# ria8651/octree-tracer

Hardware: AMD Instinct MI355X
Metric: Mrays/sec at 1920x1080, depth-16 SVO; achieved HBM GB/s vs peak (higher is better)
Workload: dtype f32+u32

## Files before the change

include/svo_hip.h:

```cpp
#ifndef SVO_HIP_H
#define SVO_HIP_H

#include <stddef.h>
#include <stdint.h>

#ifdef __cplusplus
extern "C" {
#endif

#define SVO_VOXEL_OFFSET 134217728u

typedef enum svo_status {
    SVO_OK = 0,
    SVO_ERR_ARG = -1,
    SVO_ERR_HIP = -2,
    SVO_ERR_STATE = -3,
    SVO_ERR_NO_DEVICE = -4,
    SVO_ERR_COMM = -5,
    SVO_ERR_CAP = -6
} svo_status;

#define SVO_F_PAUSE_ADAPTIVE 1u
#define SVO_F_SHOW_STEPS 2u
#define SVO_F_SHOW_HITS 4u
#define SVO_F_SHADOWS 8u
#define SVO_F_MISC_BOOL 16u

typedef struct svo_uniforms {
    float camera[16];
    float camera_inverse[16];
    float dimensions[4];
    float sun_dir[4];
    uint32_t flags;
    float misc_value;
} svo_uniforms;

typedef struct svo_hit {
    uint32_t voxel_index;
    float t;
    uint32_t steps_depth_hit;
    uint32_t packed_normal;
} svo_hit;

typedef struct svo_ctx svo_ctx;

#define SVO_VARIANT_RESTART 0
#define SVO_VARIANT_STACK 1

typedef enum svo_option {
    SVO_OPT_VARIANT = 0,
    SVO_OPT_TIMING = 1,
    SVO_OPT_GRID_BLOCKS = 2,
    SVO_OPT_REFILL_MIN = 3,
    SVO_OPT_STRIP_ITEMS = 4,
    SVO_OPT_DYNAMIC_STRIPS = 5,
    SVO_OPT_SCHEDULE = 8,
    SVO_OPT_TREE_DEPTH = 9,
    SVO_OPT_BLOCK_SHAPE = 10,
    SVO_OPT_DEBUG_BUFFER = 7,
    SVO_OPT_SCAN_CLEARS_COUNTERS = 11,
    SVO_OPT_FUSED_SHADOWS = 12,
    SVO_OPT_PAIR_TABLE = 13,
    SVO_OPT_CULL = 14,
    SVO_OPT_CAMERA_SHORTCUT = 15,
    SVO_OPT_SCHEDULE_MOTION = 16,
    SVO_OPT_PRIO_STEPS = 6
} svo_option;

int svo_device_count(void);
int svo_ctx_create(int hip_device, svo_ctx **out);
int svo_ctx_destroy(svo_ctx *ctx);
int svo_ctx_set_stream(svo_ctx *ctx, void *hip_stream, int use_own);
int svo_set_option(svo_ctx *ctx, int option, int64_t value);
const char *svo_last_error(const svo_ctx *ctx);
int svo_sync(svo_ctx *ctx);

int svo_nodes_alloc(svo_ctx *ctx, size_t capacity_words);
int svo_nodes_bind_device(svo_ctx *ctx, uint32_t *device_words, size_t capacity_words);
int svo_nodes_share(svo_ctx *ctx, svo_ctx *owner);
int svo_nodes_invalidate(svo_ctx *ctx);
int svo_nodes_write(svo_ctx *ctx, size_t word_offset, const uint32_t *host_words, size_t n);
int svo_nodes_scatter(svo_ctx *ctx, const uint32_t *indices, const uint32_t *host_words, size_t n);
int svo_nodes_read(svo_ctx *ctx, size_t word_offset, uint32_t *host_words, size_t n);
int svo_nodes_device_ptr(svo_ctx *ctx, uint32_t **out, size_t *capacity_words);

int svo_buffer_alloc(svo_ctx *ctx, size_t bytes, void **device_out);
int svo_buffer_free(svo_ctx *ctx, void *device_ptr);
int svo_buffer_read(svo_ctx *ctx, const void *device_ptr, void *host_out, size_t bytes);
int svo_buffer_write(svo_ctx *ctx, void *device_dst, const void *host_src, size_t bytes);

int svo_set_uniforms(svo_ctx *ctx, const svo_uniforms *u);

int svo_render(svo_ctx *ctx, uint32_t width, uint32_t height, uint32_t x0, uint32_t y0,
               uint32_t tile_w, uint32_t tile_h, svo_hit *hits_out, uint32_t *rgba_out);
int svo_render_host(svo_ctx *ctx, uint32_t width, uint32_t height, uint32_t x0, uint32_t y0,
                    uint32_t tile_w, uint32_t tile_h, svo_hit *hits_out, uint32_t *rgba_out);
int svo_render_tiles(svo_ctx *ctx, uint32_t width, uint32_t height, uint32_t tile_w,
                     uint32_t tile_h, uint32_t first_tile, uint32_t tile_stride,
                     svo_hit *hits_out, uint32_t *rgba_out);
int svo_render_secondary(svo_ctx *ctx, uint32_t width, uint32_t height, uint32_t x0, uint32_t y0,
                         uint32_t tile_w, uint32_t tile_h, uint32_t n_secondary, svo_hit *primary_out,
                         svo_hit *secondary_out);
int svo_render_tiles_secondary(svo_ctx *ctx, uint32_t width, uint32_t height, uint32_t tile_w,
                               uint32_t tile_h, uint32_t first_tile, uint32_t tile_stride,
                               uint32_t n_secondary, svo_hit *primary_out, svo_hit *secondary_out);
int svo_assemble_tiles(svo_ctx *ctx, const svo_hit *gathered, uint32_t world, uint32_t n_pad, uint32_t width,
                       uint32_t height, uint32_t tile_w, uint32_t tile_h, svo_hit *frame_out);
int svo_pack_records(svo_ctx *ctx, const svo_hit *records, size_t n, uint32_t *wire_out);
int svo_assemble_tiles_packed(svo_ctx *ctx, const uint32_t *gathered_wire, uint32_t world, uint32_t n_pad, uint32_t width,
                              uint32_t height, uint32_t tile_w, uint32_t tile_h, svo_hit *frame_out);
#define SVO_COMM_ID_BYTES 128
int svo_comm_unique_id(uint8_t id_out[SVO_COMM_ID_BYTES]);
int svo_comm_init_rank(svo_ctx *ctx, const uint8_t id[SVO_COMM_ID_BYTES], int world, int rank);
int svo_comm_init_all(int n, svo_ctx *const *ctxs);
int svo_comm_destroy(svo_ctx *ctx);
int svo_gather_frame(svo_ctx *ctx, const void *send, size_t bytes, void *recv_on_root, int root);
int svo_gather_wait(svo_ctx *ctx);
int svo_gather_frame_all(int n, svo_ctx *const *ctxs, const void *const *send, size_t bytes, void *recv_on_root, int root);

int svo_assemble_tiles_rgba(svo_ctx *ctx, const uint32_t *gathered_rgba, uint32_t world, uint32_t n_pad, uint32_t width,
                            uint32_t height, uint32_t tile_w, uint32_t tile_h, uint32_t *rgba_frame_out);

int svo_trace_rays(svo_ctx *ctx, const float *rays, size_t n_rays, svo_hit *hits_out);

int svo_last_render_ms(svo_ctx *ctx, float *ms);
int svo_timing_collect(svo_ctx *ctx, float *ms_out, size_t cap, size_t *n_out);

int svo_diag_gather(svo_ctx *ctx, uint32_t stride_bytes, uint32_t n_loads);

int svo_diag_strip_classes(svo_ctx *ctx, uint8_t *host_out, size_t n_strips);

int svo_scan_dispatch(svo_ctx *ctx, uint32_t node_length);
int svo_scan_read(svo_ctx *ctx, uint32_t *sub, uint32_t *n_sub, uint32_t *unsub, uint32_t *n_unsub,
                  size_t capacity);

struct svo_cpu_octree;
struct svo_world;
typedef struct svo_proc_params {
    float pos[3];
    uint32_t base_depth;
    uint32_t chunk_depth;
    uint64_t max_nodes;
} svo_proc_params;
int svo_proc_generate_chunk(svo_ctx *ctx, const svo_proc_params *params, struct svo_cpu_octree **out);
int svo_world_generate(svo_ctx *ctx, struct svo_world *w, uint32_t world_depth, uint32_t chunk_depth);
int svo_proc_sdf(svo_ctx *ctx, const float *xyz, size_t n, float *out);
int svo_proc_classify(svo_ctx *ctx, const svo_proc_params *params, uint8_t *cells_out);
#define SVO_PROC_TIMES 10
int svo_proc_timing(svo_ctx *ctx, float ms_out[SVO_PROC_TIMES]);

typedef struct svo_build_params {
    uint32_t depth;
    uint32_t default_colour;
    uint64_t max_words;
} svo_build_params;
int svo_nodes_build(svo_ctx *ctx, const uint32_t *xyz, const uint32_t *colours, size_t n, const svo_build_params *p,
                    uint64_t *n_words_out);
int svo_nodes_build_dense(svo_ctx *ctx, const uint32_t *grid, const svo_build_params *p, uint64_t *n_words_out);
#define SVO_BUILD_TIMES 6
int svo_build_timing(svo_ctx *ctx, float ms_out[SVO_BUILD_TIMES]);

typedef struct svo_edit_params {
    uint32_t depth;
    uint32_t default_colour;
    uint64_t n_words;
    uint64_t max_words;
} svo_edit_params;
int svo_nodes_edit(svo_ctx *ctx, const uint32_t *xyz, const uint32_t *colours, size_t n, const svo_edit_params *p,
                   uint64_t *n_words_out);
#define SVO_EDIT_TIMES 6
int svo_edit_timing(svo_ctx *ctx, float ms_out[SVO_EDIT_TIMES]);

#define SVO_COMPACT_PRUNE_EMPTY 1u
typedef struct svo_compact_params {
    uint32_t flags;
    uint32_t reserved;
    uint64_t n_words;
} svo_compact_params;
int svo_nodes_compact(svo_ctx *ctx, const svo_compact_params *p, uint32_t *perm_out_dev , uint64_t *n_words_out);
#define SVO_COMPACT_TIMES 6
int svo_compact_timing(svo_ctx *ctx, float ms_out[SVO_COMPACT_TIMES]);

#define SVO_LIST_EXPAND 1u
typedef struct svo_list_params {
    uint32_t flags;
    uint32_t depth;
    uint64_t n_words;
    uint64_t max_voxels;
} svo_list_params;
int svo_nodes_list_voxels(svo_ctx *ctx, const svo_list_params *p, uint32_t *xyz_out_dev, uint32_t *value_out_dev,
                          uint32_t *level_out_dev , uint64_t *n_out);
#define SVO_LIST_TIMES 5
int svo_list_timing(svo_ctx *ctx, float ms_out[SVO_LIST_TIMES]);

#define SVO_SAMPLE_FINER   (1u << 28)
#define SVO_SAMPLE_OUTSIDE (1u << 29)
#define SVO_SAMPLE_BROKEN  (1u << 30)
typedef struct svo_sample_params {
    uint32_t flags;
    uint32_t depth;
    uint64_t n_words;
} svo_sample_params;
int svo_nodes_sample(svo_ctx *ctx, const svo_sample_params *p, const uint32_t *xyz_dev, size_t n,
                     uint32_t *value_out_dev, uint32_t *level_out_dev , uint32_t *index_out_dev );
int svo_nodes_sample_dense(svo_ctx *ctx, const svo_sample_params *p, const uint32_t origin[3], const uint32_t size[3],
                           uint32_t *grid_out_dev);
#define SVO_SAMPLE_TIMES 2
int svo_sample_timing(svo_ctx *ctx, float ms_out[SVO_SAMPLE_TIMES]);

typedef struct svo_voxelize_params {
    uint32_t depth;
    uint32_t flags;
    uint32_t default_colour;
    uint32_t n_vertices;
// ... 51 lines not shown
```

octree-tracer_amd/_lib.py:

```python
import ctypes as C
import os

import torch

_HERE = os.path.dirname(os.path.abspath(__file__))
LIB_PATH = os.environ.get("SVO_HIP_LIB") or os.path.join(_HERE, "libsvo_hip.so")


class Uniforms(C.Structure):
    _fields_ = [
        ("camera", C.c_float * 16),
        ("camera_inverse", C.c_float * 16),
        ("dimensions", C.c_float * 4),
        ("sun_dir", C.c_float * 4),
        ("flags", C.c_uint32),
        ("misc_value", C.c_float),
    ]


class TerrainParams(C.Structure):
    _fields_ = [
        ("seed", C.c_uint32),
        ("max_depth", C.c_uint32),
        ("cam", C.c_float * 3),
# ... 49 lines not shown
class SampleParams(C.Structure):
    _fields_ = [
        ("flags", C.c_uint32),
        ("depth", C.c_uint32),
        ("n_words", C.c_uint64),
    ]


class VoxelizeParams(C.Structure):
    _fields_ = [
        ("depth", C.c_uint32),
        ("flags", C.c_uint32),
        ("default_colour", C.c_uint32),
        ("n_vertices", C.c_uint32),
        ("max_voxels", C.c_uint64),
    ]


class ChunkBuildParams(C.Structure):
    _fields_ = [
        ("depth", C.c_uint32),
        ("world_depth", C.c_uint32),
        ("default_colour", C.c_uint32),
        ("max_nodes", C.c_uint64),
    ]


class AdaptiveResult(C.Structure):
    _fields_ = [
        ("n_sub", C.c_uint32),
        ("n_unsub", C.c_uint32),
        ("chunks_loaded", C.c_uint64),
        ("length", C.c_uint64),
        ("n_removed", C.c_uint32),
        ("removed", C.POINTER(C.c_uint32)),
    ]


vp, sz, u32, u64, i64, f32 = C.c_void_p, C.c_size_t, C.c_uint32, C.c_uint64, C.c_int64, C.c_float
cp = C.c_char_p
fp = C.POINTER(C.c_float)

DEVICE_SIGNATURES = {
    "svo_device_count": (C.c_int, ()),
    "svo_buffer_alloc": (C.c_int, (vp, sz, C.POINTER(vp))),
    "svo_buffer_free": (C.c_int, (vp, vp)),
    "svo_buffer_read": (C.c_int, (vp, vp, vp, sz)),
    "svo_ctx_create": (C.c_int, (C.c_int, C.POINTER(vp))),
    "svo_ctx_destroy": (C.c_int, (vp,)),
    "svo_ctx_set_stream": (C.c_int, (vp, vp, C.c_int)),
    "svo_set_option": (C.c_int, (vp, C.c_int, i64)),
    "svo_last_error": (cp, (vp,)),
    "svo_sync": (C.c_int, (vp,)),
    "svo_nodes_alloc": (C.c_int, (vp, sz)),
    "svo_nodes_bind_device": (C.c_int, (vp, vp, sz)),
    "svo_nodes_write": (C.c_int, (vp, sz, vp, sz)),
    "svo_nodes_scatter": (C.c_int, (vp, vp, vp, sz)),
    "svo_nodes_read": (C.c_int, (vp, sz, vp, sz)),
    "svo_nodes_device_ptr": (C.c_int, (vp, C.POINTER(vp), C.POINTER(sz))),
    "svo_nodes_share": (C.c_int, (vp, vp)),
    "svo_nodes_invalidate": (C.c_int, (vp,)),
    "svo_comm_unique_id": (C.c_int, (vp,)),
    "svo_comm_init_rank": (C.c_int, (vp, vp, C.c_int, C.c_int)),
    "svo_comm_init_all": (C.c_int, (C.c_int, C.POINTER(vp))),
    "svo_comm_destroy": (C.c_int, (vp,)),
    "svo_gather_frame": (C.c_int, (vp, vp, sz, vp, C.c_int)),
    "svo_gather_wait": (C.c_int, (vp,)),
    "svo_gather_frame_all": (C.c_int, (C.c_int, C.POINTER(vp), C.POINTER(vp), sz, vp, C.c_int)),
    "svo_set_uniforms": (C.c_int, (vp, C.POINTER(Uniforms))),
    "svo_render": (C.c_int, (vp, u32, u32, u32, u32, u32, u32, vp, vp)),
    "svo_render_host": (C.c_int, (vp, u32, u32, u32, u32, u32, u32, vp, vp)),
    "svo_render_tiles": (C.c_int, (vp, u32, u32, u32, u32, u32, u32, vp, vp)),
    "svo_render_secondary": (C.c_int, (vp, u32, u32, u32, u32, u32, u32, u32, vp, vp)),
    "svo_render_tiles_secondary": (C.c_int, (vp, u32, u32, u32, u32, u32, u32, u32, vp, vp)),
    "svo_assemble_tiles": (C.c_int, (vp, vp, u32, u32, u32, u32, u32, u32, vp)),
    "svo_assemble_tiles_packed": (C.c_int, (vp, vp, u32, u32, u32, u32, u32, u32, vp)),
    "svo_assemble_tiles_rgba": (C.c_int, (vp, vp, u32, u32, u32, u32, u32, u32, vp)),
    "svo_pack_records": (C.c_int, (vp, vp, sz, vp)),
    "svo_trace_rays": (C.c_int, (vp, vp, sz, vp)),
    "svo_last_render_ms": (C.c_int, (vp, fp)),
    "svo_timing_collect": (C.c_int, (vp, fp, sz, C.POINTER(sz))),
    "svo_diag_gather": (C.c_int, (vp, u32, u32)),
    "svo_diag_strip_classes": (C.c_int, (vp, vp, sz)),
    "svo_scan_dispatch": (C.c_int, (vp, u32)),
    "svo_scan_read": (C.c_int, (vp, vp, C.POINTER(u32), vp, C.POINTER(u32), sz)),
    "svo_proc_generate_chunk": (C.c_int, (vp, C.POINTER(ProcParams), C.POINTER(vp))),
    "svo_world_generate": (C.c_int, (vp, vp, u32, u32)),
    "svo_proc_sdf": (C.c_int, (vp, vp, sz, vp)),
    "svo_proc_classify": (C.c_int, (vp, C.POINTER(ProcParams), vp)),
    "svo_proc_timing": (C.c_int, (vp, fp)),
    "svo_nodes_build": (C.c_int, (vp, vp, vp, sz, C.POINTER(BuildParams), C.POINTER(u64))),
    "svo_nodes_build_dense": (C.c_int, (vp, vp, C.POINTER(BuildParams), C.POINTER(u64))),
    "svo_buffer_write": (C.c_int, (vp, vp, vp, sz)),
    "svo_build_timing": (C.c_int, (vp, fp)),
    "svo_cpu_octree_build": (C.c_int, (vp, vp, vp, sz, C.POINTER(ChunkBuildParams), C.POINTER(vp))),
    "svo_world_build": (C.c_int, (vp, vp, vp, vp, sz, C.POINTER(ChunkBuildParams))),
    "svo_world_build_timing": (C.c_int, (vp, fp)),
    "svo_nodes_edit": (C.c_int, (vp, vp, vp, sz, C.POINTER(EditParams), C.POINTER(u64))),
    "svo_edit_timing": (C.c_int, (vp, fp)),
    "svo_nodes_compact": (C.c_int, (vp, C.POINTER(CompactParams), vp, C.POINTER(u64))),
    "svo_compact_timing": (C.c_int, (vp, fp)),
    "svo_nodes_list_voxels": (C.c_int, (vp, C.POINTER(ListParams), vp, vp, vp, C.POINTER(u64))),
    "svo_list_timing": (C.c_int, (vp, fp)),
    "svo_nodes_sample": (C.c_int, (vp, C.POINTER(SampleParams), vp, sz, vp, vp, vp)),
    "svo_nodes_sample_dense": (C.c_int, (vp, C.POINTER(SampleParams), C.POINTER(u32), C.POINTER(u32), vp)),
    "svo_sample_timing": (C.c_int, (vp, fp)),
    "svo_mesh_voxelize": (C.c_int, (vp, C.POINTER(VoxelizeParams), vp, vp, vp, sz, vp, vp, vp, C.POINTER(u64))),
    "svo_voxelize_timing": (C.c_int, (vp, fp)),
    "svo_adaptive_attach": (C.c_int, (vp, vp, vp)),
    "svo_adaptive_step": (C.c_int, (vp, vp, u32, vp, u32, C.POINTER(AdaptiveResult))),
    "svo_adaptive_download": (C.c_int, (vp, vp)),
    "svo_adaptive_length": (C.c_int, (vp, C.POINTER(u64))),
    "svo_adaptive_timing": (C.c_int, (vp, fp)),
    "svo_adaptive_expand": (C.c_int, (vp, u32, fp, f32, u64, C.POINTER(AdaptiveResult))),
    "svo_adaptive_expand_timing": (C.c_int, (vp, fp)),
}
HOST_SIGNATURES = {
    "svo_cpu_octree_new": (vp, (C.c_uint8,)),
    "svo_cpu_octree_free": (None, (vp,)),
    "svo_cpu_octree_len": (sz, (vp,)),
    "svo_cpu_octree_load_file": (vp, (cp, u32, cp, sz)),
    "svo_cpu_octree_load_vox": (vp, (cp, sz, cp, sz)),
    "svo_cpu_octree_load_rsvo": (vp, (cp, sz, u32, cp, sz)),
    "svo_cpu_octree_from_voxels": (vp, (u32, vp, sz, vp, cp, sz)),
    "svo_cpu_octree_put_in_voxel": (None, (vp, fp, C.POINTER(C.c_uint8), u32)),
    "svo_cpu_octree_put_in_block": (None, (vp, fp, u32, u32)),
    "svo_cpu_octree_find_voxel": (None, (vp, fp, i64, C.POINTER(u64), C.POINTER(u32), fp)),
    "svo_cpu_octree_get_node_mask": (None, (vp, sz, C.POINTER(C.c_uint8))),
    "svo_cpu_octree_to_octree": (None, (vp, vp)),
    "svo_cpu_octree_raw": (None, (vp, vp, vp)),
    "svo_cpu_octree_generate_mips": (None, (vp, C.POINTER(C.c_uint8))),
    "svo_vox_parse": (i64, (cp, sz, C.POINTER(u32), vp, sz, vp, cp, sz)),
    "svo_vox_write": (sz, (u32, vp, sz, vp, vp, sz)),
    "svo_rsvo_write": (sz, (vp, vp, sz)),
    "svo_octree_new": (vp, (C.POINTER(C.c_uint8),)),
    "svo_octree_from_words": (vp, (vp, sz)),
    "svo_octree_free": (None, (vp,)),
    "svo_octree_len": (sz, (vp,)),
    "svo_octree_raw_data": (vp, (vp,)),
    "svo_octree_get_node": (u32, (vp, sz)),
    "svo_octree_subdivide": (C.c_int, (vp, sz, C.POINTER(C.c_uint8), u32)),
    "svo_octree_unsubdivide": (C.c_int, (vp, sz)),
    "svo_octree_find_voxel": (None, (vp, fp, i64, C.POINTER(u64), C.POINTER(u32), fp)),
    "svo_octree_expanded": (C.c_int, (vp, sz, vp)),
    "svo_octree_pos_offset": (None, (u32, u32, fp)),
    "svo_octree_holes": (sz, (vp,)),
    "svo_octree_set_node": (None, (vp, sz, u32)),
    "svo_octree_position": (None, (vp, sz, fp)),
    "svo_octree_hole_stack": (sz, (vp, vp, sz)),
    "svo_octree_positions": (sz, (vp, vp, sz)),
    "svo_octree_take_dirty": (sz, (vp, vp, vp, sz)),
    "svo_world_new": (vp, (cp,)),
    "svo_world_free": (None, (vp,)),
    "svo_world_last_error": (cp, (vp,)),
    "svo_world_insert": (C.c_int, (vp, u32, vp)),
    "svo_world_remove": (C.c_int, (vp, u32)),
    "svo_world_chunk": (vp, (vp, u32)),
    "svo_world_chunk_ids": (sz, (vp, vp, sz)),
    "svo_world_find_voxel": (C.c_int, (vp, fp, i64, C.POINTER(u32), C.POINTER(u64), C.POINTER(u32), fp)),
    "svo_world_generate_mip_tree": (C.c_int, (vp, u32, C.POINTER(C.c_uint8))),
    "svo_world_save_chunk": (C.c_int, (vp, u32)),
    "svo_world_load_chunk": (C.c_int, (vp, u32)),
    "svo_world_load": (vp, (cp, cp, sz)),
    "svo_cpu_octree_bin": (sz, (vp, vp, sz)),
    "svo_cpu_octree_from_bin": (vp, (cp, sz, cp, sz)),
    "svo_adaptive_subdivide": (i64, (vp, vp, vp, sz, C.POINTER(u64))),
# ... 36 lines not shown
```

octree-tracer_amd/csrc/svo_abi.cpp:

```cpp
#include <hip/hip_runtime.h>

#include <array>
#include <cmath>
#include <cstdio>
#include <cstdlib>
#include <cstring>
#include <new>
#include <string>
#include <vector>

#include "svo_ctx.h"

int svo_fail(svo_ctx *ctx, int code, const char *what) {
    if (ctx) ctx->err = what;
    return code;
}

int svo_fail_hip(svo_ctx *ctx, hipError_t e, const char *what) {
    if (ctx) ctx->err = std::string(what) + ": " + hipGetErrorString(e);
    return SVO_ERR_HIP;
}

namespace {

// ... 70 lines not shown
    const double o[3] = {ci[12] / w, ci[13] / w, ci[14] / w};
    if (!(fabs(o[0]) > 1.001 || fabs(o[1]) > 1.001 || fabs(o[2]) > 1.001)) return false;
    if (ctx->cull_mode == 1) return true;
    constexpr int NX = 12, NY = 8;
    int miss = 0;
    for (int j = 0; j < NY; j++)
        for (int i = 0; i < NX; i++) {
            const double cx = (i + 0.5) / NX * 2.0 - 1.0, cy = -((j + 0.5) / NY * 2.0 - 1.0);
            double d4[4];
            for (int r = 0; r < 4; r++) d4[r] = ci[r] * cx + ci[4 + r] * cy + ci[8 + r] + ci[12 + r];
            if (!(fabs(d4[3]) > 1e-20)) return false;
            double t0 = -1e300, t1 = 1e300;
            for (int k = 0; k < 3; k++) {
                const double d = d4[k] / d4[3] - o[k];
                if (d == 0.0) {
                    if (fabs(o[k]) > 1.0) t1 = -1e300;
                    continue;
                }
                const double a = (-1.0 - o[k]) / d, b = (1.0 - o[k]) / d;
                t0 = fmax(t0, fmin(a, b));
                t1 = fmin(t1, fmax(a, b));
            }
            if (!(t1 >= 0.0 && t0 <= t1)) miss++;
        }
    return miss * 10 >= NX * NY * 4;
}

struct TraceOpts {
    float *aux_t = nullptr;
    bool count_rays = false;
    int sched_slot = 0;
    const uint8_t *skip = nullptr;
    svo_hit *shadow_out = nullptr;
};

svo::TraceArgs trace_args(const svo_ctx *ctx, const svo::WorkDesc &work, svo_hit *hits) {
    svo::TraceArgs a{};
    a.nodes = ctx->nodes;
    a.n_words = (uint32_t)ctx->capacity;
    a.u = ctx->uniforms;
    a.work = work;
    a.hits = hits;
    return a;
}

svo::WorkDesc ray_work(size_t n) {
    svo::WorkDesc w{};
    w.mode = 2;
    w.n_items = (uint32_t)n;
    w.bpr = w.bprect = w.tiles_x = 1;
    return w;
}

int schedule_before(svo_ctx *ctx, svo_ctx::Sched &sc, const svo::FrameFacts &f, svo::TraceArgs &a, uint32_t n_strips) {
    if (f.schedule && sc.cap < n_strips) {
        HIP_TRY(ctx, hipStreamSynchronize(ctx->stream));
        HIP_TRY(ctx, sc.alloc(n_strips));
    }
    const svo::TracePlan plan = svo::plan_before_trace(sc.state, f);
    if (!f.schedule) return SVO_OK;
    if (plan.reset_shares) {
        static const auto equal_shares = [] {
            std::array<uint32_t, svo::kBalanceWords> w{};
            for (uint32_t k = 0; k <= 8; k++) w[k] = k * 8192u;
            return w;
        }();
        HIP_TRY(ctx, hipMemcpyAsync(sc.balance, equal_shares.data(), sizeof(equal_shares), hipMemcpyHostToDevice, ctx->stream));
    }
    a.balance = plan.feed_balance ? sc.balance : nullptr;
    a.order_cap = svo::order_list_cap(n_strips);
    if (f.filtered) {
        const uint8_t *prev = plan.prior_costs ? sc.cost : nullptr;
        if (a.skip)
            HIP_TRY(ctx, svo::launch_schedule_skipping(a, prev, sc.cls_now, sc.order, n_strips, a.order_cap, ctx->stream));
        else
            HIP_TRY(ctx, svo::launch_schedule_culling(a, prev, sc.cls_now, sc.order, n_strips, a.order_cap, ctx->stream));
        a.order = sc.order;
    } else if (plan.stored_lists) {
        a.order = sc.order;
    }
    return SVO_OK;
}

int schedule_after(svo_ctx *ctx, svo_ctx::Sched &sc, svo::FrameFacts &f, const svo::TraceArgs &a, const svo::LaunchInfo &li,
                   int sched_slot) {
    f.same_input = (a.work.mode != 2 || sched_slot == 1) && sc.built_nodes_version == ctx->store->version &&
                   memcmp(&sc.built_uniforms, &ctx->uniforms, sizeof(svo_uniforms)) == 0;
    f.moving = sc.have_prev && memcmp(&sc.prev_uniforms, &ctx->uniforms, sizeof(svo_uniforms)) != 0;
    const svo::PostPlan plan = svo::plan_after_trace(sc.state, f);
    HIP_TRY(ctx, svo::launch_post(a, li, plan, sc.buf(), ctx->stream));
    sc.prev_uniforms = ctx->uniforms;
    sc.have_prev = true;
    if (plan.rebuild) {
        sc.key = a.work;
        sc.built_uniforms = ctx->uniforms;
        sc.built_nodes_version = ctx->store->version;
    }
    return SVO_OK;
}

int trace_launch(svo_ctx *ctx, const svo::WorkDesc &work, const float *rays, svo_hit *hits, const TraceOpts &opt) {
    int rc = bind(ctx);
    if (rc) return rc;
    const bool want_stack = ctx->variant != SVO_VARIANT_RESTART && ctx->tree_depth <= (uint32_t)svo::stack_max_depth(true);
    if (want_stack) {
        rc = ensure_top_table(ctx);
        if (rc) return rc;
    } else {
        rc = order_after_last_write(ctx);
        if (rc) return rc;
    }
    const bool debug_hits = (ctx->uniforms.flags & SVO_F_PAUSE_ADAPTIVE) && (ctx->uniforms.flags & SVO_F_SHOW_HITS);
    const bool stack = want_stack && !debug_hits;
    svo::WorkDesc wd = work;
    auto magic = [](uint32_t d) -> uint32_t { return d <= 1u ? 0u : (uint32_t)(0x100000000ull / d) + 1u; };
    wd.magic_bpr = magic(wd.bpr);
    wd.magic_bprect = magic(wd.bprect);
    wd.magic_tiles_x = magic(wd.tiles_x);
    svo::TraceArgs a = trace_args(ctx, wd, hits);
    a.top_table = ctx->top_table;
    a.rays = rays;
    a.aux_t = opt.aux_t;
    a.status = ctx->status;
    a.refill_min = ctx->refill_min;
    a.cam_shortcut = ctx->cam_shortcut ? 1u : 0u;
    a.debug = ctx->debug_buf;
    a.skip = opt.skip;
    const bool counting = (work.mode != 2 || opt.count_rays) && !(ctx->uniforms.flags & SVO_F_PAUSE_ADAPTIVE);
    a.count_nodes = counting ? ctx->nodes : nullptr;
    a.shadow_hits = stack ? opt.shadow_out : nullptr;

    const uint32_t n_strips = (wd.n_items + 63u) / 64u;
    svo_ctx::Sched &sc = ctx->sched[opt.sched_slot & 1];
    svo::FrameFacts f;
    f.schedule = ctx->schedule && n_strips <= svo::kMaxScheduledStrips;
    f.filtered = f.schedule && (opt.skip != nullptr || (wd.mode != 2 && hits != nullptr && cull_worthwhile(ctx)));
    f.same_layout = memcmp(&sc.key, &wd, sizeof(wd)) == 0;
    f.mode = wd.mode;
    f.n_rects = wd.n_rects;
    f.motion_floor = ctx->motion_floor;
    f.sched_period = ctx->sched_period;
    f.balance = ctx->list_balance;
    if (stack) {
        rc = schedule_before(ctx, sc, f, a, n_strips);
        if (rc) return rc;
    }

    svo::LaunchInfo li{};
    li.variant = stack ? SVO_VARIANT_STACK : SVO_VARIANT_RESTART;
    li.grid_blocks = ctx->grid_blocks;
    li.num_cus = ctx->num_cus;
    li.strip_items = ctx->strip_items;
    li.deep_stack = ctx->tree_depth > (uint32_t)svo::stack_max_depth(false);
    li.occupancy = ctx->occupancy;
    if (stack && ctx->defer_items < wd.n_items) {
        HIP_TRY(ctx, hipStreamSynchronize(ctx->stream));
        ctx->frame_parity = 0;
        ctx->defer_items = 0;
        size_t want = wd.n_items < (1u << 16) ? (1u << 16) : wd.n_items;
        HIP_TRY(ctx, ctx->defer_buf.alloc(svo::kCounterWords + 2 * (want + 1)));
        HIP_TRY(ctx, hipMemsetAsync(ctx->defer_buf, 0, ctx->defer_buf.size() * sizeof(uint32_t), ctx->stream));
        ctx->defer_items = want;
    }
    li.counters = ctx->defer_buf;
    if (ctx->defer_buf) {
        uint32_t *lists = ctx->defer_buf + svo::kCounterWords;
        const size_t stride = ctx->defer_items + 1;
        li.defer = lists + (ctx->frame_parity ? stride : 0);
        li.next_defer_count = lists + (ctx->frame_parity ? 0 : stride);
    }
    const size_t slot = ctx->ev_slots ? (ctx->ev_count % ctx->ev_slots) : 0;
    const bool timed = ctx->ev_slots && opt.sched_slot == 0;
    if (timed) HIP_TRY(ctx, hipEventRecord(ctx->ev[slot][0], ctx->stream));
    HIP_TRY(ctx, svo::launch_trace(a, li, ctx->stream));
    if (timed) {
        HIP_TRY(ctx, hipEventRecord(ctx->ev[slot][1], ctx->stream));
        ctx->ev_count++;
    }
    if (!stack) return SVO_OK;
    rc = schedule_after(ctx, sc, f, a, li, opt.sched_slot);
    if (rc) return rc;
    ctx->frame_parity ^= 1;
    return SVO_OK;
}

bool fuse_shadow_rays(const svo_ctx *ctx) {
    const bool want = ctx->fused_shadows != 0;
    if (!want || ctx->variant == SVO_VARIANT_RESTART || ctx->tree_depth > (uint32_t)svo::stack_max_depth(true)) return false;
    const float *sd = ctx->uniforms.sun_dir;
    const float sl = sqrtf((sd[0] * sd[0] + sd[1] * sd[1]) + sd[2] * sd[2]);
    for (int k = 0; k < 3; k++) {
        float d = -(sd[k] / sl);
        if (d == 0.0f) d = 0.000001f;
        if (!(fabsf(d) >= 1.0e-11f && fabsf(d) <= 2.0f)) return false;
    }
    return true;
}

int trace_common(svo_ctx *ctx, const svo::WorkDesc &work, const float *rays, svo_hit *hits, uint32_t *rgba) {
    if (!ctx->nodes) return svo_fail(ctx, SVO_ERR_STATE, "svo_nodes_alloc / svo_nodes_bind_device not called");
    if (work.mode != 2 && !ctx->have_uniforms) return svo_fail(ctx, SVO_ERR_STATE, "svo_set_uniforms not called");
    if (!hits && !rgba) return svo_fail(ctx, SVO_ERR_ARG, "both hits_out and rgba_out are NULL");
    if (!rgba) return trace_launch(ctx, work, rays, hits, TraceOpts{});
    if (work.mode == 2) return svo_fail(ctx, SVO_ERR_ARG, "explicit rays have no pixels to shade");
    int rc = bind(ctx);
    if (rc) return rc;
    const size_t n = (size_t)work.n_rects * work.w * work.h;
    const uint32_t f = ctx->uniforms.flags;
    const bool shadows = (f & SVO_F_SHADOWS) && !(f & SVO_F_SHOW_STEPS) && !(f & SVO_F_SHOW_HITS);
    if (!hits) {
        rc = svo_grow(ctx, n, &ctx->shade_hits);
        if (rc) return rc;
        hits = ctx->shade_hits;
    }
    const bool fused = shadows && fuse_shadow_rays(ctx);
    TraceOpts primary;
    if (fused) {
        rc = svo_grow(ctx, n, &ctx->shade_shadow);
        if (rc) return rc;
        primary.shadow_out = ctx->shade_shadow;
    } else {
        rc = svo_grow(ctx, n, &ctx->shade_aux);
        if (rc) return rc;
        primary.aux_t = ctx->shade_aux;
    }
    rc = trace_launch(ctx, work, nullptr, hits, primary);
    if (rc) return rc;
    const svo::TraceArgs a = trace_args(ctx, work, hits);
    if (shadows && !fused) {
        rc = svo_grow(ctx, n * 6, &ctx->shade_rays);
        if (rc) return rc;
        rc = svo_grow(ctx, n, &ctx->shade_shadow);
        if (rc) return rc;
        rc = svo_grow(ctx, n, &ctx->shade_skip);
        if (rc) return rc;
        HIP_TRY(ctx, svo::launch_secondary_gen(a, ctx->shade_aux, ctx->shade_rays, ctx->shade_skip, ctx->shade_shadow, 0u, 1u,
                                               (uint32_t)n, ctx->stream));
        TraceOpts shadow;
        shadow.count_rays = true;
        shadow.sched_slot = 1;
        shadow.skip = ctx->shade_skip;
        rc = trace_launch(ctx, ray_work(n), ctx->shade_rays, ctx->shade_shadow, shadow);
        if (rc) return rc;
    }
    HIP_TRY(ctx, svo::launch_shade(a, shadows ? ctx->shade_shadow.get() : nullptr, rgba, ctx->stream));
    return SVO_OK;
}

int trace_secondary(svo_ctx *ctx, const svo::WorkDesc &work, uint32_t n_secondary, svo_hit *primary, svo_hit *secondary) {
    if (!ctx->nodes) return svo_fail(ctx, SVO_ERR_STATE, "svo_nodes_alloc / svo_nodes_bind_device not called");
    if (!secondary) return svo_fail(ctx, SVO_ERR_ARG, "secondary_out is NULL");
    if (n_secondary < 1 || n_secondary > 4) return svo_fail(ctx, SVO_ERR_ARG, "n_secondary must be 1..4");
    int rc = bind(ctx);
    if (rc) return rc;
    const size_t n = (size_t)work.n_rects * work.w * work.h;
    if (n * n_secondary > (1u << 26)) return svo_fail(ctx, SVO_ERR_ARG, "too many secondary rays for one call");
    if (!primary) {
        rc = svo_grow(ctx, n, &ctx->shade_hits);
        if (rc) return rc;
        primary = ctx->shade_hits;
    }
    rc = svo_grow(ctx, n, &ctx->shade_aux);
    if (rc) return rc;
// ... 74 lines not shown
    const svo_events<2> &pair = ctx->ev[launch % ctx->ev_slots];
    HIP_TRY(ctx, hipEventSynchronize(pair[1]));
    HIP_TRY(ctx, hipEventElapsedTime(ms, pair[0], pair[1]));
    return SVO_OK;
}

}

int svo_store_order_after_write(svo_ctx *ctx) { return order_after_last_write(ctx); }
int svo_store_note_write(svo_ctx *ctx) { return note_write(ctx, true); }

hipError_t svo_ctx::Sched::alloc(uint32_t n_strips) {
    release();
    const uint32_t want = n_strips < 4096u ? 4096u : n_strips;
    const size_t cls_bytes = want + 32 + svo::kOrderHistWords * sizeof(uint32_t);
    const size_t order_words = 8 + 8 * (svo::order_list_cap(want) + 8);
    hipError_t e = cost.alloc(cls_bytes);
    if (e == hipSuccess) e = cls_now.alloc(cls_bytes);
    if (e == hipSuccess) e = order.alloc(order_words);
    if (e == hipSuccess) e = balance.alloc(svo::kBalanceWords);
    if (e == hipSuccess) cap = want;
    return e;
}

extern "C" {

int svo_device_count(void) {
    int n = 0;
    if (hipGetDeviceCount(&n) != hipSuccess) {
        (void)hipGetLastError();
        return 0;
    }
    return n;
}

int svo_buffer_alloc(svo_ctx *ctx, size_t bytes, void **device_out) {
    if (!ctx || !device_out || bytes == 0) return SVO_ERR_ARG;
    *device_out = nullptr;
    int rc = bind(ctx);
    if (rc) return rc;
    HIP_TRY(ctx, hipMalloc(device_out, bytes));
    return SVO_OK;
}

int svo_buffer_free(svo_ctx *ctx, void *device_ptr) {
    if (!ctx) return SVO_ERR_ARG;
    if (!device_ptr) return SVO_OK;
    int rc = bind(ctx);
    if (rc) return rc;
    HIP_TRY(ctx, hipStreamSynchronize(ctx->stream));
    if (ctx->comm_stream) HIP_TRY(ctx, hipStreamSynchronize(ctx->comm_stream));
    HIP_TRY(ctx, hipFree(device_ptr));
    return SVO_OK;
}

int svo_buffer_write(svo_ctx *ctx, void *device_dst, const void *host_src, size_t bytes) {
    if (!ctx || ((!device_dst || !host_src) && bytes)) return SVO_ERR_ARG;
    int rc = bind(ctx);
    if (rc || bytes == 0) return rc;
    HIP_TRY(ctx, hipMemcpyAsync(device_dst, host_src, bytes, hipMemcpyHostToDevice, ctx->stream));
    HIP_TRY(ctx, hipStreamSynchronize(ctx->stream));
    return SVO_OK;
}

int svo_buffer_read(svo_ctx *ctx, const void *device_ptr, void *host_out, size_t bytes) {
    if (!ctx || ((!device_ptr || !host_out) && bytes)) return SVO_ERR_ARG;
    int rc = bind(ctx);
    if (rc || bytes == 0) return rc;
    HIP_TRY(ctx, hipMemcpyAsync(host_out, device_ptr, bytes, hipMemcpyDeviceToHost, ctx->stream));
    HIP_TRY(ctx, hipStreamSynchronize(ctx->stream));
    return SVO_OK;
}

int svo_ctx_create(int hip_device, svo_ctx **out) {
    if (!out) return SVO_ERR_ARG;
    *out = nullptr;
    int n = 0;
    if (hipGetDeviceCount(&n) != hipSuccess || n <= 0) return SVO_ERR_NO_DEVICE;
    if (hip_device < 0 || hip_device >= n) return SVO_ERR_ARG;
    svo_ctx *ctx = new (std::nothrow) svo_ctx();
    if (!ctx) return SVO_ERR_HIP;
    ctx->device = hip_device;
    ctx->list_balance = getenv("SVO_NO_LIST_BALANCE") == nullptr;
    hipError_t e = hipSetDevice(hip_device);
    hipDeviceProp_t prop;
    if (e == hipSuccess) e = hipGetDeviceProperties(&prop, hip_device);
    if (e == hipSuccess) {
        ctx->num_cus = prop.multiProcessorCount;
        e = ctx->own_stream.create();
    }
    if (e == hipSuccess) e = ctx->top_table.alloc(svo::kTopEntries + svo::kTopAuxEntries);
    if (e == hipSuccess) e = ctx->status.alloc(1);
    if (e == hipSuccess) e = hipMemset(ctx->status, 0, sizeof(uint32_t));
    if (e != hipSuccess) {
        svo_ctx_destroy(ctx);
        return SVO_ERR_HIP;
    }
    ctx->stream = ctx->own_stream;
    *out = ctx;
    return SVO_OK;
}

int svo_ctx_destroy(svo_ctx *ctx) {
    if (!ctx) return SVO_OK;
    (void)hipSetDevice(ctx->device);
    if (ctx->stream) (void)hipStreamSynchronize(ctx->stream);
    svo_comm_release(ctx);
    delete ctx;
    return SVO_OK;
}

int svo_ctx_set_stream(svo_ctx *ctx, void *hip_stream, int use_own) {
    if (!ctx) return SVO_ERR_ARG;
    int rc = bind(ctx);
    if (rc) return rc;
    HIP_TRY(ctx, hipStreamSynchronize(ctx->stream));
    ctx->stream = use_own ? ctx->own_stream : (hipStream_t)hip_stream;
    return SVO_OK;
}

int svo_set_option(svo_ctx *ctx, int option, int64_t value) {
    if (!ctx) return SVO_ERR_ARG;
    switch (option) {
        case SVO_OPT_VARIANT:
            if (value != SVO_VARIANT_RESTART && value != SVO_VARIANT_STACK) return svo_fail(ctx, SVO_ERR_ARG, "unknown variant");
            ctx->variant = (int)value;
            return SVO_OK;
        case SVO_OPT_TIMING: {
            if (value < 0 || value > 65536) return svo_fail(ctx, SVO_ERR_ARG, "timing ring size out of range");
            int rc = bind(ctx);
            if (rc) return rc;
            HIP_TRY(ctx, hipStreamSynchronize(ctx->stream));
            while (ctx->ev.size() < (size_t)value) {
                svo_events<2> pair;
                HIP_TRY(ctx, pair.create());
                ctx->ev.push_back(std::move(pair));
            }
            ctx->ev_slots = (size_t)value;
            ctx->ev_count = 0;
            return SVO_OK;
        }
        case SVO_OPT_GRID_BLOCKS:
            if (value < 0 || value > 65535) return svo_fail(ctx, SVO_ERR_ARG, "grid_blocks out of range");
            ctx->grid_blocks = (int)value;
            return SVO_OK;
        case SVO_OPT_REFILL_MIN:
            if (value < 1 || value > 64) return svo_fail(ctx, SVO_ERR_ARG, "refill_min must be 1..64");
            ctx->refill_min = (uint32_t)value;
            return SVO_OK;
        case SVO_OPT_SCAN_CLEARS_COUNTERS:
            ctx->scan_clears = value != 0;
            return SVO_OK;
        case SVO_OPT_FUSED_SHADOWS:
            if (value < 0 || value > 2) return svo_fail(ctx, SVO_ERR_ARG, "fused shadows: 0 (off), 1 (on) or 2 (automatic)");
            ctx->fused_shadows = (int)value;
            return SVO_OK;
        case SVO_OPT_STRIP_ITEMS:
            if (value < 64 || value > 2048 || (value & 63)) return svo_fail(ctx, SVO_ERR_ARG, "strip_items must be a multiple of 64 in [64, 2048]");
            ctx->strip_items = (uint32_t)value;
            return SVO_OK;
        case SVO_OPT_DYNAMIC_STRIPS:
            return SVO_OK;
        case SVO_OPT_SCHEDULE:
            if (value < 0 || value > 1024) return svo_fail(ctx, SVO_ERR_ARG, "schedule period out of range");
            ctx->schedule = value != 0;
            if (value) ctx->sched_period = (uint32_t)value;
            ctx->sched[0].state.valid = ctx->sched[1].state.valid = false;
            return SVO_OK;
        case SVO_OPT_TREE_DEPTH:
            if (value < 1 || value > 31) return svo_fail(ctx, SVO_ERR_ARG, "tree depth must be 1..31");
            ctx->tree_depth = (uint32_t)value;
            return SVO_OK;
        case SVO_OPT_SCHEDULE_MOTION:
            if (value < 0 || (value & 15) > 12 || ((value >> 8) & 15) > 4 || (value >> 12) > 80)
                return svo_fail(ctx, SVO_ERR_ARG, "schedule motion: class floor (0..12, 0 = off) | radius (0..4) << 8 | min_count (0..80) << 12");
            ctx->motion_floor = (uint32_t)value;
            return SVO_OK;
        case SVO_OPT_CAMERA_SHORTCUT:
            ctx->cam_shortcut = value != 0;
            return SVO_OK;
        case SVO_OPT_CULL:
            if (value < 0 || value > 2) return svo_fail(ctx, SVO_ERR_ARG, "cull: 0 (off), 1 (whenever the camera is outside the cube) or 2 (automatic)");
            ctx->cull_mode = (int)value;
            return SVO_OK;
        case SVO_OPT_PAIR_TABLE:
            return SVO_OK;
        case SVO_OPT_DEBUG_BUFFER:
            ctx->debug_buf = (uint32_t *)(uintptr_t)value;
            return SVO_OK;
        case SVO_OPT_BLOCK_SHAPE:
            if (value < 0 || value > 6) return svo_fail(ctx, SVO_ERR_ARG, "block width log2 must be 0..6");
            ctx->block_w_log2 = (uint32_t)value;
            return SVO_OK;
        case SVO_OPT_PRIO_STEPS:
            if (value < 0 || value > 255) return svo_fail(ctx, SVO_ERR_ARG, "prio_steps must be 0..255");
            return SVO_OK;
        default:
            return svo_fail(ctx, SVO_ERR_ARG, "unknown option");
    }
}

const char *svo_last_error(const svo_ctx *ctx) { return ctx ? ctx->err.c_str() : "null ctx"; }

int svo_sync(svo_ctx *ctx) {
    if (!ctx) return SVO_ERR_ARG;
    int rc = bind(ctx);
    if (rc) return rc;
    HIP_TRY(ctx, hipStreamSynchronize(ctx->stream));
    if (ctx->comm_stream) HIP_TRY(ctx, hipStreamSynchronize(ctx->comm_stream));
    uint32_t st = 0;
    HIP_TRY(ctx, hipMemcpy(&st, ctx->status, sizeof(st), hipMemcpyDeviceToHost));
    if (st & 2u) {
        HIP_TRY(ctx, hipMemset(ctx->status, 0, sizeof(uint32_t)));
        return svo_fail(ctx, SVO_ERR_STATE, "fused shadow ray outside the range of the fast arithmetic (set SVO_OPT_FUSED_SHADOWS to 0)");
    }
    if (st & 1u) {
        HIP_TRY(ctx, hipMemset(ctx->status, 0, sizeof(uint32_t)));
        return svo_fail(ctx, SVO_ERR_STATE,
                        "octree deeper than SVO_OPT_TREE_DEPTH declares (the frame's records are not valid); "
                        "raise SVO_OPT_TREE_DEPTH (above 22: the general kernel) or use SVO_VARIANT_RESTART");
    }
    return SVO_OK;
}

int svo_nodes_alloc(svo_ctx *ctx, size_t capacity_words) {
    if (!ctx) return SVO_ERR_ARG;
    int rc = adopt_new_store(ctx, nullptr, capacity_words);
    if (rc) return rc;
    HIP_TRY(ctx, hipMemsetAsync(ctx->nodes, 0, capacity_words * sizeof(uint32_t), ctx->stream));
    return note_write(ctx, true);
}

int svo_nodes_bind_device(svo_ctx *ctx, uint32_t *device_words, size_t capacity_words) {
    if (!ctx || !device_words) return SVO_ERR_ARG;
    return adopt_new_store(ctx, device_words, capacity_words);
}

int svo_nodes_share(svo_ctx *ctx, svo_ctx *owner) {
    if (!ctx || !owner) return SVO_ERR_ARG;
    if (!owner->store) return svo_fail(ctx, SVO_ERR_STATE, "the owner has no node buffer (svo_nodes_alloc / svo_nodes_bind_device)");
    if (owner->device != ctx->device) return svo_fail(ctx, SVO_ERR_ARG, "contexts on different devices cannot share a node buffer");
    if (ctx->store == owner->store) return SVO_OK;
    int rc = bind(ctx);
    if (rc) return rc;
    HIP_TRY(ctx, hipStreamSynchronize(ctx->stream));
    release_store(ctx);
    adopt_store(ctx, owner->store);
    return SVO_OK;
}

int svo_nodes_invalidate(svo_ctx *ctx) {
    if (!ctx) return SVO_ERR_ARG;
    if (!ctx->store) return svo_fail(ctx, SVO_ERR_STATE, "svo_nodes_alloc / svo_nodes_bind_device not called");
    int rc = bind(ctx);
    if (rc) return rc;
    return note_write(ctx, true);
}

int svo_nodes_write(svo_ctx *ctx, size_t word_offset, const uint32_t *host_words, size_t n) {
    if (!ctx || (!host_words && n)) return SVO_ERR_ARG;
    if (!ctx->nodes) return svo_fail(ctx, SVO_ERR_STATE, "svo_nodes_alloc not called");
    if (word_offset > ctx->capacity || n > ctx->capacity - word_offset)
        return svo_fail(ctx, SVO_ERR_ARG, "write past the node buffer capacity");
    int rc = bind(ctx);
    if (rc) return rc;
    if (n) {
        rc = order_after_last_write(ctx);
        if (rc) return rc;
        HIP_TRY(ctx, hipMemcpyAsync(ctx->nodes + word_offset, host_words, n * sizeof(uint32_t), hipMemcpyHostToDevice,
                                    ctx->stream));
    }
    return note_write(ctx, true);
}

int svo_nodes_scatter(svo_ctx *ctx, const uint32_t *indices, const uint32_t *host_words, size_t n) {
    if (!ctx || ((!indices || !host_words) && n)) return SVO_ERR_ARG;
    if (!ctx->nodes) return svo_fail(ctx, SVO_ERR_STATE, "svo_nodes_alloc not called");
    if (n > (1u << 28)) return svo_fail(ctx, SVO_ERR_ARG, "too many words for one scatter");
    for (size_t i = 0; i < n; i++)
// ... 105 lines not shown
                           uint32_t height, uint32_t tile_w, uint32_t tile_h, svo_hit *frame_out) {
    if (!ctx || !gathered || !frame_out) return SVO_ERR_ARG;
    if (world == 0 || tile_w == 0 || tile_h == 0 || width % tile_w || height % tile_h)
        return svo_fail(ctx, SVO_ERR_ARG, "frame must be a whole number of tiles");
    const uint64_t tiles = (uint64_t)(width / tile_w) * (height / tile_h);
    if ((uint64_t)n_pad * world < tiles) return svo_fail(ctx, SVO_ERR_ARG, "gathered buffer holds fewer tiles than the frame");
    if ((uint64_t)width * height > (1u << 26)) return svo_fail(ctx, SVO_ERR_ARG, "frame too large");
    int rc = bind(ctx);
    if (rc) return rc;
    HIP_TRY(ctx, svo::launch_assemble_tiles(gathered, packed, frame_out, world, n_pad, width, height, tile_w, tile_h, ctx->stream));
    return SVO_OK;
}

int svo_assemble_tiles(svo_ctx *ctx, const svo_hit *gathered, uint32_t world, uint32_t n_pad, uint32_t width, uint32_t height,
                       uint32_t tile_w, uint32_t tile_h, svo_hit *frame_out) {
    return assemble_common(ctx, gathered, false, world, n_pad, width, height, tile_w, tile_h, frame_out);
}

int svo_assemble_tiles_packed(svo_ctx *ctx, const uint32_t *gathered_wire, uint32_t world, uint32_t n_pad, uint32_t width,
                              uint32_t height, uint32_t tile_w, uint32_t tile_h, svo_hit *frame_out) {
    return assemble_common(ctx, gathered_wire, true, world, n_pad, width, height, tile_w, tile_h, frame_out);
}

int svo_assemble_tiles_rgba(svo_ctx *ctx, const uint32_t *gathered_rgba, uint32_t world, uint32_t n_pad, uint32_t width, uint32_t height,
                            uint32_t tile_w, uint32_t tile_h, uint32_t *rgba_frame_out) {
    if (!ctx || !gathered_rgba || !rgba_frame_out) return SVO_ERR_ARG;
    if (world == 0 || tile_w == 0 || tile_h == 0 || width % tile_w || height % tile_h)
        return svo_fail(ctx, SVO_ERR_ARG, "frame must be a whole number of tiles");
    const uint64_t tiles = (uint64_t)(width / tile_w) * (height / tile_h);
    if ((uint64_t)n_pad * world < tiles) return svo_fail(ctx, SVO_ERR_ARG, "gathered buffer holds fewer tiles than the frame");
    if ((uint64_t)width * height > (1u << 26)) return svo_fail(ctx, SVO_ERR_ARG, "frame too large");
    int rc = bind(ctx);
    if (rc) return rc;
    HIP_TRY(ctx, svo::launch_assemble_tiles_rgba(gathered_rgba, rgba_frame_out, world, n_pad, width, height, tile_w, tile_h, ctx->stream));
    return SVO_OK;
}

int svo_pack_records(svo_ctx *ctx, const svo_hit *records, size_t n, uint32_t *wire_out) {
    if (!ctx || ((!records || !wire_out) && n)) return SVO_ERR_ARG;
    if (n > (1u << 26)) return svo_fail(ctx, SVO_ERR_ARG, "too many records for one call");
    int rc = bind(ctx);
    if (rc) return rc;
    HIP_TRY(ctx, svo::launch_pack_records(records, wire_out, (uint32_t)n, ctx->stream));
    return SVO_OK;
}

int svo_trace_rays(svo_ctx *ctx, const float *rays, size_t n_rays, svo_hit *hits_out) {
    if (!ctx || (!rays && n_rays)) return SVO_ERR_ARG;
    if (n_rays > (1u << 26)) return svo_fail(ctx, SVO_ERR_ARG, "too many rays for one call");
    return trace_common(ctx, ray_work(n_rays), rays, hits_out, nullptr);
}

int svo_last_render_ms(svo_ctx *ctx, float *ms) {
    if (!ctx || !ms) return SVO_ERR_ARG;
    if (!ctx->ev_slots || !ctx->ev_count) return svo_fail(ctx, SVO_ERR_STATE, "no timed launch (set SVO_OPT_TIMING first)");
    int rc = bind(ctx);
    if (rc) return rc;
    return timed_launch_ms(ctx, ctx->ev_count - 1, ms);
}

int svo_timing_collect(svo_ctx *ctx, float *ms_out, size_t cap, size_t *n_out) {
    if (!ctx || !n_out || (!ms_out && cap)) return SVO_ERR_ARG;
    *n_out = 0;
    if (!ctx->ev_slots) return svo_fail(ctx, SVO_ERR_STATE, "timing is off (set SVO_OPT_TIMING first)");
    int rc = bind(ctx);
    if (rc) return rc;
    size_t n = ctx->ev_count < ctx->ev_slots ? ctx->ev_count : ctx->ev_slots;
    if (n > cap) n = cap;
    const size_t first = ctx->ev_count - n;
    for (size_t i = 0; i < n; i++)
        if ((rc = timed_launch_ms(ctx, first + i, &ms_out[i]))) return rc;
    *n_out = n;
    ctx->ev_count = 0;
    return SVO_OK;
}

int svo_diag_gather(svo_ctx *ctx, uint32_t stride_bytes, uint32_t n_loads) {
    if (!ctx || stride_bytes < 4 || (stride_bytes & 3)) return SVO_ERR_ARG;
    if (!ctx->nodes) return svo_fail(ctx, SVO_ERR_STATE, "svo_nodes_alloc not called");
    if ((uint64_t)n_loads * (stride_bytes / 4) > ctx->capacity) return svo_fail(ctx, SVO_ERR_ARG, "pattern exceeds the node buffer");
    int rc = bind(ctx);
    if (rc) return rc;
    HIP_TRY(ctx, svo::launch_diag_gather(ctx->nodes, (uint32_t)ctx->capacity, stride_bytes / 4, n_loads, ctx->status, ctx->stream));
    return SVO_OK;
}

int svo_diag_strip_classes(svo_ctx *ctx, uint8_t *host_out, size_t n_strips) {
    if (!ctx || (!host_out && n_strips)) return SVO_ERR_ARG;
    const svo_ctx::Sched &sc = ctx->sched[0];
    if (!sc.cls_now || !sc.state.order_filtered) return svo_fail(ctx, SVO_ERR_STATE, "the last pixel frame was traced without a culling pass");
    if (n_strips > sc.cap) return svo_fail(ctx, SVO_ERR_ARG, "more strips than the last frame had");
    int rc = bind(ctx);
    if (rc || n_strips == 0) return rc;
    HIP_TRY(ctx, hipMemcpyAsync(host_out, sc.cls_now, n_strips, hipMemcpyDeviceToHost, ctx->stream));
    HIP_TRY(ctx, hipStreamSynchronize(ctx->stream));
    return SVO_OK;
}

int svo_scan_dispatch(svo_ctx *ctx, uint32_t node_length) {
    if (!ctx) return SVO_ERR_ARG;
    if (!ctx->nodes) return svo_fail(ctx, SVO_ERR_STATE, "svo_nodes_alloc not called");
    int rc = bind(ctx);
    if (rc) return rc;
    if (!ctx->scan_lists) {
        HIP_TRY(ctx, ctx->scan_lists.alloc(2 * kScanCapacity));
        ctx->scan_capacity = kScanCapacity;
        HIP_TRY(ctx, hipMemsetAsync(ctx->scan_sub(), 0, sizeof(uint32_t), ctx->stream));
        HIP_TRY(ctx, hipMemsetAsync(ctx->scan_unsub(), 0, sizeof(uint32_t), ctx->stream));
    }
    uint32_t n = node_length < ctx->capacity ? node_length : (uint32_t)ctx->capacity;
    rc = order_after_last_write(ctx);
    if (rc) return rc;
    HIP_TRY(ctx, svo::launch_scan(ctx->nodes, n, node_length, ctx->scan_sub(), ctx->scan_unsub(),
                                  (uint32_t)ctx->scan_capacity, ctx->scan_clears, ctx->stream));
    return SVO_OK;
}

int svo_scan_read(svo_ctx *ctx, uint32_t *sub, uint32_t *n_sub, uint32_t *unsub, uint32_t *n_unsub, size_t capacity) {
    if (!ctx || !sub || !unsub || !n_sub || !n_unsub || capacity < 1) return SVO_ERR_ARG;
    if (!ctx->scan_lists) return svo_fail(ctx, SVO_ERR_STATE, "svo_scan_dispatch not called");
    int rc = bind(ctx);
    if (rc) return rc;
    uint32_t counts[2] = {0, 0};
    HIP_TRY(ctx, hipMemcpyAsync(&counts[0], ctx->scan_sub(), sizeof(uint32_t), hipMemcpyDeviceToHost, ctx->stream));
    HIP_TRY(ctx, hipMemcpyAsync(&counts[1], ctx->scan_unsub(), sizeof(uint32_t), hipMemcpyDeviceToHost, ctx->stream));
    HIP_TRY(ctx, hipStreamSynchronize(ctx->stream));
    uint32_t ls = counts[0] < ctx->scan_capacity - 1 ? counts[0] : (uint32_t)ctx->scan_capacity - 1;
    uint32_t lu = counts[1] < ctx->scan_capacity - 1 ? counts[1] : (uint32_t)ctx->scan_capacity - 1;
    if (ls + 1 > capacity) ls = (uint32_t)capacity - 1;
    if (lu + 1 > capacity) lu = (uint32_t)capacity - 1;
    sub[0] = ls;
    unsub[0] = lu;
    if (ls) HIP_TRY(ctx, hipMemcpyAsync(sub + 1, ctx->scan_sub() + 1, ls * sizeof(uint32_t), hipMemcpyDeviceToHost, ctx->stream));
    if (lu) HIP_TRY(ctx, hipMemcpyAsync(unsub + 1, ctx->scan_unsub() + 1, lu * sizeof(uint32_t), hipMemcpyDeviceToHost, ctx->stream));
    HIP_TRY(ctx, hipMemsetAsync(ctx->scan_sub(), 0, sizeof(uint32_t), ctx->stream));
    HIP_TRY(ctx, hipMemsetAsync(ctx->scan_unsub(), 0, sizeof(uint32_t), ctx->stream));
    HIP_TRY(ctx, hipStreamSynchronize(ctx->stream));
    *n_sub = ls;
    *n_unsub = lu;
    return SVO_OK;
}

}
```

octree-tracer_amd/csrc/svo_ctx.h:

```cpp
#pragma once
#include <hip/hip_runtime.h>

#include <algorithm>
#include <chrono>
#include <cstdint>
#include <cstring>
#include <memory>
#include <string>
#include <type_traits>
#include <utility>
#include <vector>

#include "svo_device.h"
#include "svo_hip.h"
#include "svo_host.h"


template <typename T, bool kPinned>
struct svo_mem {
    T *p = nullptr;
    size_t n = 0;
    svo_mem() = default;
    svo_mem(svo_mem &&o) noexcept : p(o.p), n(o.n) { o.p = nullptr, o.n = 0; }
    svo_mem &operator=(svo_mem &&o) noexcept {
        std::swap(p, o.p);
        std::swap(n, o.n);
        return *this;
    }
    ~svo_mem() { reset(); }
    void reset() {
        if (p) (void)(kPinned ? hipHostFree(p) : hipFree(p));
        p = nullptr;
        n = 0;
    }
    hipError_t alloc(size_t items) {
        reset();
        const size_t bytes = items * sizeof(std::conditional_t<std::is_void<T>::value, char, T>);
        const hipError_t e = kPinned ? hipHostMalloc((void **)&p, bytes, hipHostMallocDefault) : hipMalloc((void **)&p, bytes);
        if (e == hipSuccess) n = items;
        else p = nullptr;
        return e;
    }
    size_t size() const { return n; }
    T *get() const { return p; }
    operator T *() const { return p; }
    T *operator->() const { return p; }
};
template <typename T>
using svo_dev = svo_mem<T, false>;
template <typename T>
using svo_pinned = svo_mem<T, true>;

template <int N>
struct svo_events {
    hipEvent_t e[N] = {};
    svo_events() = default;
    svo_events(svo_events &&o) noexcept {
        for (int k = 0; k < N; k++) e[k] = o.e[k], o.e[k] = nullptr;
    }
    svo_events &operator=(const svo_events &) = delete;
    ~svo_events() { reset(); }
    void reset() {
        for (hipEvent_t &x : e) {
            if (x) (void)hipEventDestroy(x);
            x = nullptr;
        }
    }
    hipError_t create(unsigned flags = hipEventDefault) {
        for (hipEvent_t &x : e)
            if (!x)
                if (hipError_t err = flags ? hipEventCreateWithFlags(&x, flags) : hipEventCreate(&x)) return err;
        return hipSuccess;
    }
    hipEvent_t operator[](int k) const { return e[k]; }
};

struct svo_stream {
    hipStream_t s = nullptr;
    svo_stream() = default;
    svo_stream(const svo_stream &) = delete;
    svo_stream &operator=(const svo_stream &) = delete;
    ~svo_stream() { reset(); }
    void reset() {
        if (s) (void)hipStreamDestroy(s);
        s = nullptr;
    }
    hipError_t create() { return hipStreamCreateWithFlags(&s, hipStreamNonBlocking); }
    operator hipStream_t() const { return s; }
};

struct svo_node_store {
    int device = 0;
    uint32_t *nodes = nullptr;
    size_t capacity = 0;
    bool owned = false;
    uint64_t version = 1;
    svo_events<1> last_write;
    hipStream_t last_writer = nullptr;
    ~svo_node_store() {
        (void)hipSetDevice(device);
        if (nodes && owned) (void)hipFree(nodes);
    }
};

struct svo_proc_state;
struct svo_build_state;
struct svo_adapt_state;
struct svo_edit_state;
struct svo_compact_state;
struct svo_list_state;
struct svo_sample_state;
struct svo_voxelize_state;
template <typename T>
using svo_workspace = std::unique_ptr<T, void (*)(T *)>;
template <typename T>
svo_workspace<T> svo_workspace_new() {
    return svo_workspace<T>(new T(), [](T *p) { delete p; });
}

struct svo_ctx {
    svo_stream own_stream;
    svo_stream comm_stream;
    int device = 0;
    int num_cus = 256;
    hipStream_t stream = nullptr;
    std::shared_ptr<svo_node_store> store;
    uint32_t *nodes = nullptr;
    size_t capacity = 0;
    uint64_t top_version = 0;
    svo_dev<uint32_t> top_table;
    int cull_mode = 2;
    bool cam_shortcut = true;
    void *comm = nullptr;
    int comm_world = 0, comm_rank = 0;
    svo_events<2> comm_ev;
    bool gathers_issued = false;
    svo_dev<uint32_t> status;
    svo_dev<uint32_t> defer_buf;
    size_t defer_items = 0;
    svo_dev<uint32_t> scan_lists;
    size_t scan_capacity = 0;
    uint32_t *scan_sub() const { return scan_lists; }
    uint32_t *scan_unsub() const { return scan_lists + scan_capacity; }
    svo_dev<char> stage;
    svo_uniforms uniforms{};
    bool have_uniforms = false;
    int variant = SVO_VARIANT_STACK;
    int grid_blocks = 0;
    int occupancy[16] = {};
    uint32_t refill_min = 32;
    bool scan_clears = false;
    int fused_shadows = 2;
    svo_dev<uint32_t> scatter_buf;
    uint32_t block_w_log2 = 3;
    uint32_t tree_depth = 16;
    struct Sched {
        svo::SchedState state;
        svo_dev<uint8_t> cost, cls_now;
        svo_dev<uint32_t> order, balance;
        size_t cap = 0;
        svo::SchedBuffers buf() const { return {cost, cls_now, order, balance}; }
        svo::WorkDesc key{};
        svo_uniforms built_uniforms{};
        uint64_t built_nodes_version = 0;
        svo_uniforms prev_uniforms{};
        bool have_prev = false;
        hipError_t alloc(uint32_t n_strips);
        void release() { *this = Sched{}; }
    };
    Sched sched[2];
    bool list_balance = true;
    uint32_t motion_floor = 0x1204;
    bool schedule = true;
    uint32_t sched_period = 2;
    int frame_parity = 0;
    svo_dev<svo_hit> shade_hits, shade_shadow;
    svo_dev<float> shade_aux, shade_rays;
    svo_dev<uint8_t> shade_skip;
    uint32_t *debug_buf = nullptr;
    uint32_t strip_items = 64;
    std::vector<svo_events<2>> ev;
    size_t ev_slots = 0, ev_count = 0;
    svo_workspace<svo_proc_state> proc{nullptr, nullptr};
    svo_workspace<svo_build_state> build{nullptr, nullptr};
    svo_workspace<svo_adapt_state> adapt{nullptr, nullptr};
    svo_workspace<svo_edit_state> edit{nullptr, nullptr};
    svo_workspace<svo_compact_state> compact{nullptr, nullptr};
    svo_workspace<svo_list_state> list{nullptr, nullptr};
    svo_workspace<svo_sample_state> sample{nullptr, nullptr};
    svo_workspace<svo_voxelize_state> voxelize{nullptr, nullptr};
    std::string err;
};


int svo_fail(svo_ctx *ctx, int code, const char *what);
int svo_fail_hip(svo_ctx *ctx, hipError_t e, const char *what);
inline int svo_fail(svo_ctx *ctx, int code, const std::string &what) { return svo_fail(ctx, code, what.c_str()); }

#define HIP_TRY(ctx, expr)                                          \
    do {                                                            \
        hipError_t e_ = (expr);                                     \
        if (e_ != hipSuccess) return svo_fail_hip(ctx, e_, #expr); \
    } while (0)

inline double svo_now_ms() {
    return std::chrono::duration<double, std::milli>(std::chrono::steady_clock::now().time_since_epoch()).count();
}

inline uint32_t svo_div_up(uint64_t n, uint64_t per) { return (uint32_t)((n + per - 1) / per); }


template <bool kPinned, typename... T>
int svo_grow_group(svo_ctx *ctx, size_t want, svo_mem<T, kPinned> *...bufs) {
    if (std::min({bufs->size()...}) >= want) return SVO_OK;
    HIP_TRY(ctx, hipStreamSynchronize(ctx->stream));
    (bufs->reset(), ...);
    hipError_t group_alloc = hipSuccess;
    (void)(... && ((group_alloc = bufs->alloc(want)) == hipSuccess));
    HIP_TRY(ctx, group_alloc);
    return SVO_OK;
}
template <typename... T>
int svo_grow(svo_ctx *ctx, size_t want, svo_dev<T> *...bufs) { return svo_grow_group(ctx, want, bufs...); }
template <typename... T>
int svo_grow_pinned(svo_ctx *ctx, size_t want, svo_pinned<T> *...bufs) { return svo_grow_group(ctx, want, bufs...); }

template <typename T>
int svo_grow_keep(svo_ctx *ctx, size_t want, svo_dev<T> *buf, size_t keep) {
    if (buf->size() >= want) return SVO_OK;
    svo_dev<T> bigger;
    HIP_TRY(ctx, bigger.alloc(want));
    if (keep) HIP_TRY(ctx, hipMemcpyAsync(bigger, *buf, keep * sizeof(T), hipMemcpyDeviceToDevice, ctx->stream));
    HIP_TRY(ctx, hipStreamSynchronize(ctx->stream));
    *buf = std::move(bigger);
    return SVO_OK;
}

template <typename T = uint32_t>
struct svo_mirrored {
    svo_dev<T> dev;
    svo_pinned<T> mirror;
    int alloc(svo_ctx *ctx, size_t items) {
        HIP_TRY(ctx, mirror.alloc(items));
        HIP_TRY(ctx, dev.alloc(items));
        return SVO_OK;
    }
    hipError_t zero(svo_ctx *ctx) { return hipMemsetAsync(dev, 0, dev.size() * sizeof(T), ctx->stream); }
    hipError_t copy(svo_ctx *ctx, size_t items = ~size_t(0)) {
        return hipMemcpyAsync(mirror, dev, std::min(items, dev.size()) * sizeof(T), hipMemcpyDeviceToHost, ctx->stream);
    }
    int read(svo_ctx *ctx, size_t items = ~size_t(0)) {
        HIP_TRY(ctx, copy(ctx, items));
        HIP_TRY(ctx, hipStreamSynchronize(ctx->stream));
// ... 122 lines not shown
```

octree-tracer_amd/csrc/svo_device.h:

```cpp
#pragma once
#include <hip/hip_runtime.h>
#include <stdint.h>

#include "svo_hip.h"
#include "svo_sched.h"

namespace svo {

constexpr uint32_t kVoxelOffset = 134217728u;
constexpr uint32_t kMaxDescent = 31;
constexpr int kTopLevels = 3;
constexpr int kTopEntries = 1 << (3 * kTopLevels);
constexpr int kTopAuxEntries = 8 + 64;
constexpr int kPathBits = 23;
#ifndef SVO_COUNTER_STRIDE
#define SVO_COUNTER_STRIDE 16416
#endif
constexpr int kCounterStride = SVO_COUNTER_STRIDE;
constexpr int kCounterWords = 64 * kCounterStride;


struct WorkDesc {
    uint32_t mode;
    uint32_t x0, y0;
    uint32_t w, h;
    uint32_t bw_log2;
    uint32_t bpr;
    uint32_t bprect;
    uint32_t n_rects;
    uint32_t tiles_x;
    uint32_t first_tile, tile_stride;
    uint32_t n_items;
    uint32_t magic_bpr, magic_bprect, magic_tiles_x;
};

struct TraceArgs {
    const uint32_t *nodes;
    uint32_t n_words;
    const uint32_t *top_table;
    svo_uniforms u;
    WorkDesc work;
    const float *rays;
    svo_hit *hits;
    uint32_t *rgba;
    float *aux_t;
    uint32_t *status;
    uint32_t refill_min;
    uint32_t cam_shortcut;
    uint32_t *count_nodes;
    const uint32_t *order;
    uint32_t order_cap;
    uint32_t *debug;
    const uint8_t *skip;
    uint32_t *balance;
    svo_hit *shadow_hits;
};

struct LaunchInfo {
    int variant;
    int grid_blocks;
    int num_cus;
    int *occupancy;
    bool deep_stack;
    uint32_t strip_items;
    uint32_t *counters;
    uint32_t *defer;
    uint32_t *next_defer_count;
};

hipError_t launch_build_top_table(const uint32_t *nodes, uint32_t n_words, uint32_t *top_table,
                                  hipStream_t stream);
hipError_t launch_trace(const TraceArgs &args, const LaunchInfo &li, hipStream_t stream);
int stack_max_depth(bool deep);
constexpr uint32_t kMaxScheduledStrips = 1u << 20;
#ifndef SVO_COST_SHIFT
#define SVO_COST_SHIFT 2
#endif
constexpr uint32_t kCostShift = SVO_COST_SHIFT, kCostClasses = 128u >> SVO_COST_SHIFT;
constexpr uint32_t kOrderHistWords = 64 * kCostClasses;
constexpr uint32_t kBalanceStart = 9;
constexpr uint32_t kBalanceUpdates = 18;
constexpr uint32_t kBalanceStamps = 19;
constexpr uint32_t kBalanceBestTime = 20;
constexpr uint32_t kBalanceBestShares = 21;
constexpr uint32_t kBalanceHead = 32, kBalanceSlots = 4096, kBalanceWords = kBalanceHead + kBalanceSlots;
inline uint32_t order_list_cap(uint32_t n_strips) { return (n_strips + 3u) / 4u + kCostClasses; }
struct SchedBuffers {
    uint8_t *cost;
    uint8_t *cls_now;
    uint32_t *order;
    uint32_t *balance;
};
hipError_t launch_post(const TraceArgs &args, const LaunchInfo &li, const PostPlan &plan, const SchedBuffers &buf, hipStream_t stream);
hipError_t launch_build_lists(const TraceArgs &args, uint32_t motion_floor, const SchedBuffers &buf, hipStream_t stream);

hipError_t launch_schedule_skipping(const TraceArgs &args, const uint8_t *prev, uint8_t *cls, uint32_t *sched, uint32_t n_strips,
                                    uint32_t cap, hipStream_t stream);
hipError_t launch_schedule_culling(const TraceArgs &args, const uint8_t *prev, uint8_t *cls, uint32_t *sched, uint32_t n_strips,
                                   uint32_t cap, hipStream_t stream);
hipError_t launch_secondary_gen(const TraceArgs &args, const float *aux_t, float *rays, uint8_t *skip, svo_hit *out, uint32_t k_first,
                                uint32_t n_secondary, uint32_t n_records, hipStream_t stream);
hipError_t launch_shade(const TraceArgs &args, const svo_hit *shadow_hits, uint32_t *rgba, hipStream_t stream);
hipError_t launch_diag_gather(const uint32_t *buf, uint32_t n_words, uint32_t stride_words, uint32_t n_loads, uint32_t *sink,
                              hipStream_t stream);
hipError_t launch_scan(uint32_t *nodes, uint32_t n_words, uint32_t node_length, uint32_t *sub, uint32_t *unsub,
                       uint32_t capacity, bool clear_counters, hipStream_t stream);
hipError_t launch_assemble_tiles(const void *gathered, bool packed, svo_hit *frame, uint32_t world, uint32_t n_pad, uint32_t width,
                                 uint32_t height, uint32_t tile_w, uint32_t tile_h, hipStream_t stream);
hipError_t launch_assemble_tiles_rgba(const uint32_t *gathered, uint32_t *frame, uint32_t world, uint32_t n_pad, uint32_t width,
                                      uint32_t height, uint32_t tile_w, uint32_t tile_h, hipStream_t stream);
hipError_t launch_pack_records(const svo_hit *records, uint32_t *wire, uint32_t n, hipStream_t stream);
hipError_t launch_scatter(uint32_t *nodes, uint32_t n_words, const uint32_t *indices, const uint32_t *words, uint32_t n,
                          hipStream_t stream);

}
```

octree-tracer_amd/csrc/svo_kernels.hip:

```cpp
#include <hip/hip_runtime.h>

#include "svo_device.h"
#include "svo_trace_fn.h"

#ifndef SVO_DBG_LIGHT
#define SVO_DBG_LIGHT 0
#endif
#ifndef SVO_WAVES_PER_SIMD_CNT
#define SVO_WAVES_PER_SIMD_CNT 6
#endif
#ifndef SVO_WAVES_PER_SIMD
#define SVO_WAVES_PER_SIMD 7
#endif

namespace svo {


__device__ __forceinline__ uint32_t count_add(uint32_t *nodes, uint32_t p, uint32_t word, uint32_t n) {
    while ((word & 15u) < 15u) {
        const uint32_t add = min(n, 15u - (word & 15u));
        const uint32_t seen = atomicCAS(&nodes[p], word, word + add);
        if (seen == word) return (word & 15u) + add;
        word = seen;
    }
// ... 109 lines not shown
            write_hit(hits, out, 0xFF000000u, dist + t_current, steps, 100u, 1u,
                      normal_code(n0) | (normal_code(n1) << 2) | (normal_code(n2) << 4));
            if (aux) aux[out] = t_current;
            return t_current;
        }
    }
}


__device__ __forceinline__ float trace_one_restart(const TraceArgs &a, rsrc_t rs, bool misc_bool, bool counter_hits, uint32_t q) {
    Item it = decode_item(a.work, q);
    if (!it.valid) return 0.0f;
    if (a.work.mode == 2 && a.skip && a.skip[q]) return 0.0f;
    return trace_ray_restart(a, rs, misc_bool, counter_hits, item_ray(a, it), a.hits, it.out, a.aux_t);
}

__global__ __launch_bounds__(256) void trace_restart_kernel(TraceArgs a, const uint32_t *list) {
    const rsrc_t rs = make_rsrc(a.nodes, a.n_words);
    const bool misc_bool = (a.u.flags & SVO_F_MISC_BOOL) != 0;
    const bool counter_hits = (a.u.flags & SVO_F_PAUSE_ADAPTIVE) && (a.u.flags & SVO_F_SHOW_HITS);
    const uint32_t n = list ? list[0] : a.work.n_items;
    for (uint32_t i = blockIdx.x * 256u + threadIdx.x; i < n; i += gridDim.x * 256u)
        trace_one_restart(a, rs, misc_bool, counter_hits, list ? list[1u + i] : i);
}

__global__ __launch_bounds__(256) void build_top_table_kernel(const uint32_t *nodes, uint32_t n_words,
                                                              uint32_t *table, int top_levels) {
    const rsrc_t rs = make_rsrc(nodes, n_words);
    uint32_t cell = blockIdx.x * 256u + threadIdx.x;
    if (cell >= (1u << (3 * top_levels))) return;
    uint32_t cx = (cell >> (2 * top_levels)) & ((1u << top_levels) - 1u);
    uint32_t cy = (cell >> top_levels) & ((1u << top_levels) - 1u);
    uint32_t cz = cell & ((1u << top_levels) - 1u);
    uint32_t node_index = 0, entry = ((uint32_t)top_levels + 1u) << 27;
    for (int lvl = 1; lvl <= top_levels; lvl++) {
        int sh = top_levels - lvl;
        uint32_t child = (((cx >> sh) & 1u) << 2) | (((cy >> sh) & 1u) << 1) | ((cz >> sh) & 1u);
        uint32_t tn = load_word(rs, node_index + child) >> 4;
        if (tn >= kVoxelOffset) {
            entry = ((uint32_t)lvl << 27) | (node_index & 0x07FFFFFFu);
            break;
        }
        node_index = tn;
        entry = (((uint32_t)top_levels + 1u) << 27) | (tn & 0x07FFFFFFu);
    }
    table[cell] = entry;
    uint32_t at = (uint32_t)kTopEntries;
    for (int k = 1; k < top_levels; k++) {
        if (cell < (1u << (3 * k))) {
            const uint32_t kx = (cell >> (2 * k)) & ((1u << k) - 1u), ky = (cell >> k) & ((1u << k) - 1u), kz = cell & ((1u << k) - 1u);
            uint32_t g = 0;
            for (int lvl = 1; lvl <= k && g != 0xFFFFFFFFu; lvl++) {
                const int sh = k - lvl;
                const uint32_t child = (((kx >> sh) & 1u) << 2) | (((ky >> sh) & 1u) << 1) | ((kz >> sh) & 1u);
                const uint32_t tn = load_word(rs, g + child) >> 4;
                g = tn >= kVoxelOffset ? 0xFFFFFFFFu : tn;
            }
            table[at + cell] = g;
        }
        at += 1u << (3 * k);
    }
}


__device__ __forceinline__ const TraceArgs &fresh_args() {
    auto p = (const __attribute__((address_space(4))) char *)__builtin_amdgcn_kernarg_segment_ptr();
    asm volatile("" : "+s"(p));
    return *(const TraceArgs *)p;
}

template <int BLOCK, int NS, int K, bool CNT>
struct StackLds {
    static constexpr int top = 1 << (3 * K);
    static constexpr int lut = top;
    static constexpr int pools = lut + 64;
    static constexpr int counting = pools + (BLOCK / 64) * (kPoolWords * 64);
    static constexpr int stacks = counting + (CNT ? (BLOCK / 64) * kCountQueue + kSatTags + (1 << (3 * K)) / 8 : 0);
    static constexpr int total = stacks + NS * BLOCK;
};
#if defined(__HIP_DEVICE_COMPILE__) && !defined(__gfx950__)
#error "svo_kernels.hip is written for gfx950: the walk relies on its handling of LDS accesses beyond the allocation and on v_rcp_f32 + one Newton step being the IEEE reciprocal (tools/rcptest_gpu.hip)"
#endif

template <int BLOCK, int NS, int K, bool GE, bool DBG, bool CNT, bool SHD>
__global__ __launch_bounds__(BLOCK, NS > 12 ? 4 : (CNT ? SVO_WAVES_PER_SIMD_CNT : ((SHD || (DBG && SVO_DBG_LIGHT == 0)) ? 6 : SVO_WAVES_PER_SIMD))) void trace_stack_kernel(TraceArgs a, uint32_t strip_items,
                                                               uint32_t *work_counter, uint32_t *defer) {
    constexpr bool DBGH = DBG && SVO_DBG_LIGHT == 0;
    constexpr int D = kPathBits;
    constexpr int SBASE = K + 2;
    constexpr int SMAX = K + 1 + NS;
    static_assert(SMAX <= D - 1, "stack deeper than the path codes");
    constexpr int TBL = 1 << (3 * K);
    using Lds = StackLds<BLOCK, NS, K, CNT>;
    constexpr int kLutWords = 64;
    constexpr int LOFF = Lds::lut;
    constexpr int TOFF = Lds::pools;
    constexpr bool kLut = NS <= 12;
    constexpr int SOFF = Lds::stacks;
    static_assert(Lds::total == SOFF + NS * BLOCK, "the ancestor stacks are the last LDS region (see StackLds)");
    static_assert(D == 23, "2^D + code must be an f32 with unit spacing");
    constexpr float kScale = (float)(1 << (D - 1));
    constexpr float kInvScale = 1.0f / kScale;
    constexpr float kMagic = (float)(1 << D);
    constexpr float kNudge = 0.000002f * kScale;
    float shadow_d0 = 0.0f, shadow_d1 = 0.0f, shadow_d2 = 0.0f;
    float sDr0 = 1.0f, sDr1 = 1.0f, sDr2 = 1.0f, sY0 = 1.0f, sY1 = 1.0f, sY2 = 1.0f;
    float sS0 = 1.0f, sS1 = 1.0f, sS2 = 1.0f;
    if (SHD) {
        auto uni = [](float x) { return __uint_as_float(__builtin_amdgcn_readfirstlane(__float_as_uint(x))); };
        float sun[3];
        sun_direction(a.u, sun);
        shadow_d0 = uni(-sun[0]); shadow_d1 = uni(-sun[1]); shadow_d2 = uni(-sun[2]);
        sDr0 = uni((shadow_d0 + ((shadow_d0 == 0.0f) ? 1.0f : 0.0f) * 0.000001f) * kScale);
        sDr1 = uni((shadow_d1 + ((shadow_d1 == 0.0f) ? 1.0f : 0.0f) * 0.000001f) * kScale);
        sDr2 = uni((shadow_d2 + ((shadow_d2 == 0.0f) ? 1.0f : 0.0f) * 0.000001f) * kScale);
        sY0 = uni(1.0f / sDr0); sY1 = uni(1.0f / sDr1); sY2 = uni(1.0f / sDr2);
        sS0 = uni(copysign_bits(1.0f, sDr0)); sS1 = uni(copysign_bits(1.0f, sDr1)); sS2 = uni(copysign_bits(1.0f, sDr2));
    }
    extern __shared__ uint32_t lds[];
    uint32_t *pool_all = lds + TOFF;
    const uint32_t *aux = a.top_table + TBL;

    const uint32_t tid = threadIdx.x;
    const uint32_t lane = tid & 63u;
    uint32_t *pool = pool_all + (tid >> 6) * (kPoolWords * 64);
    const rsrc_t rs = make_rsrc(a.nodes, a.n_words);
    typedef uint32_t u32x4 __attribute__((ext_vector_type(4)));
    const u32x4 rs_asm = {(uint32_t)__builtin_amdgcn_readfirstlane((int)(uint32_t)(uintptr_t)a.nodes),
                          (uint32_t)__builtin_amdgcn_readfirstlane((int)(uint32_t)((uintptr_t)a.nodes >> 32)) & 0xFFFFu,
                          (uint32_t)__builtin_amdgcn_readfirstlane((int)(a.n_words << 2)), 0x00020000u};
    uint32_t c_refill = 0, c_desc = 0, c_step = 0, c_gen = 0, dbg_desc_iters = 0, dbg_desc_lanes = 0, dbg_desc_rounds = 0, dbg_desc_start = 0;
    uint32_t *cq = pool_all + (BLOCK / 64) * (kPoolWords * 64) + (tid >> 6) * kCountQueue;
    uint32_t *sat_tags = pool_all + (BLOCK / 64) * (kPoolWords * 64) + (BLOCK / 64) * kCountQueue;
    auto sat_slot = [](uint32_t p) -> uint32_t { return (p ^ (p >> 9)) & (uint32_t)(kSatTags - 1); };
    uint32_t *top_sat = sat_tags + kSatTags;
    if (CNT) {
        for (uint32_t i = tid; i < (uint32_t)kSatTags; i += BLOCK) sat_tags[i] = 0xFFFFFFFFu;
        for (uint32_t i = tid; i < (uint32_t)(TBL / 8); i += BLOCK) top_sat[i] = 0u;
        __syncthreads();
    }
    uint32_t cq_n = 0u;
    static_assert(kCountQueue == 128, "the flush holds the queue in two registers per lane");
    auto cq_flush = [&]() {
        constexpr uint32_t kFree = 0xFFFFFFFFu, kWord = 0x07FFFFFFu;
        const bool v0 = lane < cq_n, v1 = 64u + lane < cq_n;
        const uint32_t rec0 = v0 ? cq[lane] : 0u, rec1 = v1 ? cq[64u + lane] : 0u;
        cq[lane] = kFree;
        cq[64u + lane] = kFree;
        auto merge_in = [&](bool valid, uint32_t rec, uint32_t &slot) -> bool {
            const uint32_t p = rec & kWord;
            slot = (p * 2654435761u) >> 25;
            uint32_t role = valid ? 0u : 3u;
            uint32_t seen = 0u;
#pragma unroll
            for (int t = 0; t < 4; t++) {
                if (role == 0u) {
                    seen = atomicCAS(&cq[slot], kFree, rec);
                    if (seen == kFree) role = 1u;
                    else if ((seen & kWord) == p) role = 2u;
                    else slot = (slot + 1u) & 127u;
                }
            }
            if (role == 2u) {
                for (;;) {
                    const uint32_t sum = min(15u, (seen >> 27) + (rec >> 27));
                    const uint32_t want = p | (sum << 27);
                    if (want == seen) break;
                    const uint32_t got = atomicCAS(&cq[slot], seen, want);
                    if (got == seen) break;
                    seen = got;
                }
            }
            if (role == 0u) slot = 0xFFFFFFFFu;
            return role <= 1u;
        };
        uint32_t slot0, slot1;
        const bool i0 = merge_in(v0, rec0, slot0), i1 = merge_in(v1, rec1, slot1);
        __builtin_amdgcn_wave_barrier();
        __builtin_amdgcn_fence(__ATOMIC_ACQ_REL, "wavefront");
        const uint32_t p0 = rec0 & kWord, p1 = rec1 & kWord;
        const uint32_t n0 = (i0 && slot0 != 0xFFFFFFFFu) ? cq[slot0] >> 27 : rec0 >> 27;
        const uint32_t n1 = (i1 && slot1 != 0xFFFFFFFFu) ? cq[slot1] >> 27 : rec1 >> 27;
        const uint32_t f0 = i0 ? __hip_atomic_load(a.count_nodes + p0, __ATOMIC_RELAXED, __HIP_MEMORY_SCOPE_AGENT) : 15u;
        const uint32_t f1 = i1 ? __hip_atomic_load(a.count_nodes + p1, __ATOMIC_RELAXED, __HIP_MEMORY_SCOPE_AGENT) : 15u;
        const bool t0 = (f0 & 15u) < 15u, t1 = (f1 & 15u) < 15u;
        const uint32_t a0 = min(n0, 15u - (f0 & 15u)), a1 = min(n1, 15u - (f1 & 15u));
        uint32_t s0 = f0, s1 = f1;
        if (t0) s0 = atomicCAS(&a.count_nodes[p0], f0, f0 + a0);
        if (t1) s1 = atomicCAS(&a.count_nodes[p1], f1, f1 + a1);
        uint32_t c0 = !t0 ? 15u : (s0 == f0 ? (f0 & 15u) + a0 : 16u), c1 = !t1 ? 15u : (s1 == f1 ? (f1 & 15u) + a1 : 16u);
        if (c0 == 16u) c0 = count_add(a.count_nodes, p0, s0, n0);
        if (c1 == 16u) c1 = count_add(a.count_nodes, p1, s1, n1);
        if (i0 && c0 == 15u) sat_tags[sat_slot(p0)] = p0;
        if (i1 && c1 == 15u) sat_tags[sat_slot(p1)] = p1;
        cq_n = 0u;
    };
    auto cq_push = [&](bool mine, uint32_t p, uint32_t word) {
        const uint32_t n = visit_groups<true>(a.n_words, p, mine ? word : 15u);
        const uint64_t m = __ballot(n != 0u);
        if (!m) return;
#ifndef SVO_COUNT_FLUSH_AT
#define SVO_COUNT_FLUSH_AT (kCountQueue - 64)
#endif
        if (cq_n > (uint32_t)(SVO_COUNT_FLUSH_AT)) {
            if (DBGH) dbg_desc_rounds += 1u;
            const uint64_t c_f0 = DBGH ? __builtin_amdgcn_s_memtime() : 0ull;
            cq_flush();
            if (DBGH && lane == 0u) dbg_desc_lanes += (uint32_t)(__builtin_amdgcn_s_memtime() - c_f0);
        }
        if (n) cq[cq_n + __builtin_amdgcn_mbcnt_hi((uint32_t)(m >> 32), __builtin_amdgcn_mbcnt_lo((uint32_t)m, 0u))] = p | (min(n, 15u) << 27);
        cq_n += (uint32_t)__popcll(m);
    };

    for (uint32_t i = tid; i < (uint32_t)TBL; i += BLOCK) lds[i] = a.top_table[i];
    if (kLut && tid < (uint32_t)kLutWords) {
        uint32_t sp3 = 0u;
#pragma unroll
        for (int j = 0; j < 6; j++) sp3 |= ((tid >> j) & 1u) << (3 * j);
        lds[LOFF + tid] = __float_as_uint((float)sp3);
    }
    __syncthreads();

    const uint32_t n_items = a.work.n_items;
    const uint32_t wave_id = __builtin_amdgcn_readfirstlane((blockIdx.x * BLOCK + tid) >> 6);

    constexpr uint32_t kShards = 8, kShardStride = (uint32_t)kCounterStride;
    constexpr uint32_t kSubs = 8;
    static_assert(kShards * kSubs == 64, "the stealing probe reads one counter per lane");
    const uint32_t n_strips = (n_items + strip_items - 1) / strip_items;
    const uint32_t *order = a.order;
    uint32_t home = (blockIdx.x % kShards) * kSubs + (blockIdx.x / kShards) % kSubs;
    uint32_t pend = 0;
    uint32_t next, strip_end;
    auto entry_of = [=](uint32_t sh, uint32_t k) -> uint32_t {
        if (order) return k < order[sh] ? order[kShards + sh * a.order_cap + k] : 0xFFFFFFFFu;
        const uint32_t cand = (((k >> 4) * kShards + sh) << 4) | (k & 15u);
        return cand < n_strips ? cand : 0xFFFFFFFFu;
    };
    {
        const uint32_t my_rank = (blockIdx.x / kShards) * (uint32_t)(BLOCK / 64) + __builtin_amdgcn_readfirstlane(tid >> 6);
        const uint32_t s0 = __builtin_amdgcn_readfirstlane(entry_of(blockIdx.x % kShards, my_rank));
        if (s0 != 0xFFFFFFFFu) {
            next = s0 * strip_items;
            strip_end = min(next + strip_items, n_items);
        } else {
            pend = 0x00FFFFFFu;
            next = strip_end = 0xFFFFFFFEu;
        }
    }
    uint32_t pool_n = 0, pool_i = 0;
    uint32_t t_begin = 0, t_dry = 0;
    uint32_t n_rounds = 0, dbg_active = 0, dbg_iters = 0, dbg_refills = 0, dbg_gens = 0;
    uint64_t c_mark = 0;
    if (DBG) t_begin = (uint32_t)__builtin_amdgcn_s_memrealtime();

    float stf = ST_IDLE;
    uint32_t out = 0;
    float P0 = 0, P1 = 0, P2 = 0, Dr0 = 1, Dr1 = 1, Dr2 = 1, Y0 = 1, Y1 = 1, Y2 = 1;
    float S0 = 1, S1 = 1, S2 = 1;
    float dist = 0.0f, tcur = 0.0f;
    float stepsf = 0.0f;
    float nmf = 0.0f;
    uint32_t mu0 = __float_as_uint(kMagic), mu1 = mu0, mu2 = mu0;
    uint32_t sh = __float_as_uint(kMagic + 1.0f), nidx = 0;
    auto sh_of = [](uint32_t shbits) -> uint32_t { return shbits & 31u; };
    constexpr uint32_t kShMagic = 0x4B000000u;
    constexpr uint32_t kRb = (uint32_t)(31 - D);
    constexpr uint32_t kRow = (uint32_t)(BLOCK * 4);
    const uint32_t colbase = ((uint32_t)SOFF + threadIdx.x) * 4u - (kRb + (uint32_t)SBASE) * kRow;
    uint32_t sp = colbase + (kRb + (uint32_t)SBASE) * kRow;
    uint32_t leaf_off = 0, leaf_w = 0;
    auto sabs = [](float x) -> float { return SHD ? __builtin_fabsf(x) : x; };
    constexpr bool kWalkStops = !CNT;
    constexpr bool kWalkAsm = !DBGH;
    uint32_t satm = 0;

    typedef __attribute__((address_space(3))) uint32_t lds_u32;
    auto lds_at = [&](uint32_t byte_offset) -> lds_u32 & { return *(lds_u32 *)(uintptr_t)byte_offset; };
    if (__builtin_amdgcn_groupstaticsize() != 0u) __builtin_trap();
    auto restart_at_rb = [&](uint32_t rb) {
        const bool top = rb <= (uint32_t)(K + 1) + kRb;
        sp = colbase + rb * kRow;
        if (__ballot(top)) {
            const uint32_t cell = (__builtin_amdgcn_ubfe(mu0, D - K, K) << (2 * K)) | (__builtin_amdgcn_ubfe(mu1, D - K, K) << K) |
                                  __builtin_amdgcn_ubfe(mu2, D - K, K);
            const uint32_t e = lds_at(top ? cell * 4u : sp);
            sh = (kShMagic + (uint32_t)(D + 1)) - (top ? (e >> 27) : rb - kRb);
            nidx = e & 0x07FFFFFFu;
            sp = top ? colbase + (kRb + (uint32_t)SBASE - 1u) * kRow : sp;
        } else {
            sh = (kShMagic + (uint32_t)(D + 1) + kRb) - rb;
            nidx = lds_at(sp);
        }
    };
    auto restart_at = [&](uint32_t r) { restart_at_rb(r + kRb); };

    auto flush_record = [&](bool may_continue) {
        const TraceArgs &a = fresh_args();
        const uint32_t steps = (uint32_t)stepsf;
        const bool too_deep = leaf_w < (kVoxelOffset << 4) || __uint_as_float(sh) < kMagic + (float)(D - SMAX), solid = (leaf_w >> 4) != kVoxelOffset, inb = steps == 101u;
        const bool stop_here = too_deep || solid;
        if (too_deep) atomicOr(a.status, 1u);
        const uint32_t L = (uint32_t)D - sh_of(sh), nm = (uint32_t)__builtin_fmaf(nmf, 1.0f / kNudge, 0.5f);
        uint32_t c0n = (Dr0 > 0.0f) ? 2u : 1u, c1n = (Dr1 > 0.0f) ? 2u : 1u, c2n = (Dr2 > 0.0f) ? 2u : 1u;
        uint32_t ncode = ((nm & 1u) ? c0n : 0u) | ((nm & 2u) ? (c1n << 2) : 0u) | ((nm & 4u) ? (c2n << 4) : 0u);
        if (steps == 0u) ncode = out >> 26;
        if (!stop_here && !inb) ncode = 0u;
        const uint32_t leaf_index = leaf_off >> 2;
        const uint32_t value = too_deep ? 0xFF000000u : (solid ? leaf_index : (!inb ? 0x20202000u : 0xFF000000u));
        const uint32_t depth = (too_deep || (!solid && inb)) ? 100u : L;
        const uint32_t hit = (stop_here || inb) ? 1u : 0u;
        const bool was_shadow = SHD && stf < 0.0f;
        write_hit(was_shadow ? a.shadow_hits : a.hits, out & 0x03FFFFFFu, value, dist + tcur, steps, depth, hit, ncode);
        if (a.aux_t && !was_shadow) a.aux_t[out & 0x03FFFFFFu] = tcur;
        if (SHD && !was_shadow) {
            bool go = false;
            float pos2[3], dir2[3], d2 = 0.0f;
            if (may_continue && hit) {
                const float pw[3] = {P0 * kInvScale, P1 * kInvScale, P2 * kInvScale};
                const float dw[3] = {Dr0 * kInvScale, Dr1 * kInvScale, Dr2 * kInvScale};
                float org[3], nrm[3];
                secondary_origin(pw, dw, steps, ncode, tcur, org, nrm);
// ... 155 lines not shown
#undef WALK_LUT_REFILL
#undef WALK_EXIT
#undef WALK_OUT
#undef WALK_IN
        } else {
            while ((int32_t)w >= 0 && trips != 0u) {
                trips -= 1u;
                nidx = w >> 4;
                sp += (uint32_t)(BLOCK * 4);
                asm("" : "+v"(sp));
                lds_at(sp) = nidx;
                read_word(false);
            }
        }
        sh = __float_as_uint(__uint_as_float(sh) + 1.0f);
        if (CNT && kWalkAsm && kLut) satm |= __builtin_bitreverse32(satb) >> ((sh + (uint32_t)(32 - D)) & 31u);
        const bool below = __uint_as_float(sh) < kMagic + (float)(D - SMAX);
        if (!kWalkStops) w = below ? 0u : w;
        leaf_off = off;
        leaf_w = w;
        if (kWalkStops) stf *= ((w >> 4) != kVoxelOffset || below) ? 0.25f : 0.5f;
        else stf *= 0.5f;
    };

    constexpr bool CAM = !CNT;
    uint32_t camv = 0;
    bool cam_ok = false;
    if (CAM && a.cam_shortcut && a.work.mode != 2) {
        const RayIn r0 = gen_ray(a.u, 0u, 0u);
        if (in_bounds(r0.px, r0.py, r0.pz)) {
            mu0 = entry_magic<GE>(r0.px * kScale);
            mu1 = entry_magic<GE>(r0.py * kScale);
            mu2 = entry_magic<GE>(r0.pz * kScale);
            stf = ST_DESC;
            restart_at(1u);
            descend();
            uint32_t v = lane < (uint32_t)NS ? (uint32_t)lds_at(colbase + (kRb + (uint32_t)SBASE + lane) * kRow) : 0u;
            v = lane == (uint32_t)NS ? leaf_off : v;
            v = lane == (uint32_t)NS + 1u ? leaf_w : v;
            v = lane == (uint32_t)NS + 2u ? sh : v;
            camv = v;
            cam_ok = (uint32_t)D - sh_of((uint32_t)__builtin_amdgcn_readfirstlane(sh)) >= (uint32_t)(SBASE + 2);
            stf = ST_IDLE;
        }
    }

    {
        uint32_t *const bal = fresh_args().balance;
        if (bal != nullptr && blockIdx.x == 0u && tid == 0u) {
            bal[kBalanceStart] = (uint32_t)__builtin_amdgcn_s_memrealtime();
        }
    }
    if (DBG) {
        uint32_t *const ev = fresh_args().debug + 16u * 16384u + 16u * wave_id;
        if (lane == 0u) ev[0] = (uint32_t)__builtin_amdgcn_s_memrealtime();
        if (lane == 0u) ev[15] = (((uint32_t)__builtin_amdgcn_s_getreg((4 - 1) << 11 | 0 << 6 | 20)) << 16) | (uint32_t)__builtin_amdgcn_s_getreg((16 - 1) << 11 | 0 << 6 | 4);
    }
    for (;;) {
        if (DBGH) c_mark = __builtin_amdgcn_s_memtime();
        if (DBG) n_rounds += 1;
        if (DBGH) {
            const uint32_t nd = (uint32_t)__popcll(__ballot(sabs(stf) == ST_DESC));
            (void)nd;
            if (!CNT) dbg_desc_rounds += nd ? 1u : 0u;
        }
        if (sabs(stf) == ST_DESC) {
            descend();
        }
        if (DBGH) {
            const uint64_t now = __builtin_amdgcn_s_memtime();
            c_desc += (uint32_t)(now - c_mark);
            c_mark = now;
        }
        uint64_t act = __ballot(sabs(stf) >= ST_LEAF);
        const uint32_t n_idle = 64u - (uint32_t)__popcll(act);
        if (n_idle >= a.refill_min) {
            if (next == 0xFFFFFFFEu && pool_n == 0u) {
                const uint64_t c_w0 = DBG ? __builtin_amdgcn_s_memtime() : 0ull;
                if (DBG && !DBGH) {
                    asm volatile("s_waitcnt vmcnt(0)" ::: "memory");
                    dbg_desc_rounds += (uint32_t)(__builtin_amdgcn_s_memtime() - c_w0);
                }
                uint32_t lst = home / kSubs;
                uint32_t s = entry_of(lst, __builtin_amdgcn_readfirstlane(pend) * kSubs + home % kSubs + ((gridDim.x + kShards - 1u - lst) / kShards) * (uint32_t)(BLOCK / 64));
                while (s == 0xFFFFFFFFu) {
                    if (DBG && !DBGH && lane == 0u) dbg_desc_iters += 1u;
                    const uint32_t l = lane / kSubs;
                    const uint32_t cv = __hip_atomic_load(work_counter + lane * kShardStride, __ATOMIC_RELAXED, __HIP_MEMORY_SCOPE_AGENT);
                    const uint32_t res_l = ((gridDim.x + kShards - 1u - l) / kShards) * (uint32_t)(BLOCK / 64);
                    uint32_t len_l;
                    if (order) {
                        len_l = order[l];
                    } else {
                        const uint32_t runs = (n_strips + 15u) >> 4, mine = runs > l ? (runs - l + kShards - 1u) / kShards : 0u;
                        len_l = (mine << 4) - ((runs != 0u && (runs - 1u) % kShards == l) ? (runs << 4) - n_strips : 0u);
                    }
                    const uint64_t has = __ballot((uint64_t)cv * kSubs + lane % kSubs + res_l < (uint64_t)len_l);
                    if (!has) break;
                    const uint64_t rot = home ? ((has >> home) | (has << (64u - home))) : has;
                    home = (home + (uint32_t)__ffsll((unsigned long long)rot) - 1u) & 63u;
                    lst = home / kSubs;
                    uint32_t k = 0u;
                    if (lane == 0) k = atomicAdd(work_counter + home * kShardStride, 1u);
                    s = entry_of(lst, __builtin_amdgcn_readfirstlane(k) * kSubs + home % kSubs + ((gridDim.x + kShards - 1u - lst) / kShards) * (uint32_t)(BLOCK / 64));
                }
                home = (home & ~(kSubs - 1u)) | ((home + 1u) & (kSubs - 1u));
                s = __builtin_amdgcn_readfirstlane(s);
                next = s != 0xFFFFFFFFu ? s * strip_items : 0xFFFFFFFFu;
                strip_end = s != 0xFFFFFFFFu ? min(next + strip_items, n_items) : 0xFFFFFFFFu;
                if (DBG && next == 0xFFFFFFFFu && t_dry == 0) t_dry = (uint32_t)__builtin_amdgcn_s_memrealtime() | 1u;
                if (DBG && !CNT) dbg_desc_start += (uint32_t)(__builtin_amdgcn_s_memtime() - c_w0);
            }
            const bool more = (pool_n != 0u) || (next != 0xFFFFFFFFu);
            if (more) {
                if (DBGH) dbg_refills += 1;
                if (pool_n == 0u) {
                    if (DBG) dbg_gens += 1;
                    if (DBG && dbg_gens <= 14u) {
                        uint32_t *const ev = fresh_args().debug + 16u * 16384u + 16u * wave_id + dbg_gens;
                        if (lane == 0u) ev[0] = (uint32_t)__builtin_amdgcn_s_memrealtime();
                    }
                    const uint64_t c_g0 = DBGH ? __builtin_amdgcn_s_memtime() : 0ull;
                    const TraceArgs &a = fresh_args();
                    const uint32_t q = next + lane;
                    bool alive = false;
                    float gp0 = 0, gp1 = 0, gp2 = 0, gd0 = 1, gd1 = 1, gd2 = 1, gdist = 0;
                    uint32_t gout = 0;
                    if (q < strip_end) {
                        ItemFast it = decode_item_fast(a.work, q);
                        if (a.work.mode == 2 && a.skip && a.skip[q]) it.valid = false;
                        if (it.valid) {
                            RayIn r;
                            if (a.work.mode == 2) {
                                const float *p = a.rays + 6ull * it.out;
                                r = RayIn{p[0], p[1], p[2], p[3], p[4], p[5]};
                            } else {
                                r = gen_ray(a.u, it.px, it.py);
                            }
                            float pos[3], dir[3];
                            if (!ray_enter(r, pos, dir, gdist)) {
                                write_hit(a.hits, it.out, 0u, 0.0f, 0u, 0u, 0u, 0u);
                                if (a.aux_t) a.aux_t[it.out] = 0.0f;
                                if (SHD) reinterpret_cast<uint4 *>(a.shadow_hits)[it.out] = make_uint4(0u, 0u, 0u, 0u);
                            } else if (!(clean_component(pos[0], dir[0]) && clean_component(pos[1], dir[1]) &&
                                         clean_component(pos[2], dir[2]) && fabsf(gdist) <= 1.0e30f)) {
                                uint32_t slot = atomicAdd(&defer[0], 1u);
                                defer[1u + slot] = q;
                            } else {
                                alive = true;
                                gp0 = pos[0]; gp1 = pos[1]; gp2 = pos[2];
                                gd0 = dir[0]; gd1 = dir[1]; gd2 = dir[2];
                                uint32_t ncode = normal_code(truncf(gp0 * 1.000001f)) |
                                                 (normal_code(truncf(gp1 * 1.000001f)) << 2) |
                                                 (normal_code(truncf(gp2 * 1.000001f)) << 4);
                                gout = it.out | (ncode << 26);
                            }
                        }
                    }
                    const uint64_t am = __ballot(alive);
                    if (alive) {
                        const uint32_t slot = __builtin_amdgcn_mbcnt_hi((uint32_t)(am >> 32),
                                                                        __builtin_amdgcn_mbcnt_lo((uint32_t)am, 0u));
                        gd0 *= kScale; gd1 *= kScale; gd2 *= kScale;
                        pool[0 * 64 + slot] = __float_as_uint(gp0 * kScale);
                        pool[1 * 64 + slot] = __float_as_uint(gp1 * kScale);
                        pool[2 * 64 + slot] = __float_as_uint(gp2 * kScale);
                        pool[3 * 64 + slot] = __float_as_uint(gd0);
                        pool[4 * 64 + slot] = __float_as_uint(gd1);
                        pool[5 * 64 + slot] = __float_as_uint(gd2);
                        pool[6 * 64 + slot] = __float_as_uint(gdist);
                        pool[7 * 64 + slot] = gout;
                    }
                    pool_n = (uint32_t)__popcll(am);
                    pool_i = 0u;
                    next += min(64u, strip_end - next);
                    if (next >= strip_end) {
                        if (lane == 0) pend = atomicAdd(work_counter + home * kShardStride, 1u);
#ifdef SVO_PROBE_CLAIM_LATENCY
                        if (DBG) {
                            const uint64_t c_a0 = __builtin_amdgcn_s_memtime();
                            asm volatile("s_waitcnt vmcnt(0)" ::: "memory");
                            dbg_desc_start += (uint32_t)(__builtin_amdgcn_s_memtime() - c_a0);
                        }
#endif
                        next = strip_end = 0xFFFFFFFEu;
                    }
                    if (DBG && next == 0xFFFFFFFFu && t_dry == 0) t_dry = (uint32_t)__builtin_amdgcn_s_memrealtime() | 1u;
                    if (DBGH) c_gen += (uint32_t)(__builtin_amdgcn_s_memtime() - c_g0);
                }
                if (sabs(stf) == ST_PENDING) flush_record(true);
                if (SHD) act = __ballot(sabs(stf) >= ST_LEAF);
                if (!(sabs(stf) >= ST_LEAF)) {
                    const uint64_t idle = ~act;
                    const uint32_t rank = __builtin_amdgcn_mbcnt_hi((uint32_t)(idle >> 32),
                                                                    __builtin_amdgcn_mbcnt_lo((uint32_t)idle, 0u));
                    if (rank < pool_n) {
                        const uint32_t e = pool_i + rank;
                        P0 = __uint_as_float(pool[0 * 64 + e]);
                        P1 = __uint_as_float(pool[1 * 64 + e]);
                        P2 = __uint_as_float(pool[2 * 64 + e]);
                        Dr0 = __uint_as_float(pool[3 * 64 + e]);
                        Dr1 = __uint_as_float(pool[4 * 64 + e]);
                        Dr2 = __uint_as_float(pool[5 * 64 + e]);
                        Y0 = recip_rn(Dr0);
                        Y1 = recip_rn(Dr1);
                        Y2 = recip_rn(Dr2);
                        S0 = copysign_bits(1.0f, Dr0);
                        S1 = copysign_bits(1.0f, Dr1);
                        S2 = copysign_bits(1.0f, Dr2);
                        dist = __uint_as_float(pool[6 * 64 + e]);
                        out = pool[7 * 64 + e];
                        tcur = 0.0f;
                        stepsf = 0.0f;
                        nmf = 0.0f;
                        if (CAM && cam_ok && dist == 0.0f) {
                            const uint32_t sh0 = (uint32_t)__builtin_amdgcn_readlane((int)camv, NS + 2), L0 = (uint32_t)D - sh_of(sh0);
                            for (uint32_t l = 0; l < (uint32_t)NS && l + (uint32_t)SBASE <= L0; l++)
                                lds_at(colbase + (kRb + (uint32_t)SBASE + l) * kRow) = (uint32_t)__builtin_amdgcn_readlane((int)camv, (int)l);
                            leaf_off = (uint32_t)__builtin_amdgcn_readlane((int)camv, NS);
                            leaf_w = (uint32_t)__builtin_amdgcn_readlane((int)camv, NS + 1);
                            sh = sh0;
                            mu0 = entry_magic<GE>(P0); mu1 = entry_magic<GE>(P1); mu2 = entry_magic<GE>(P2);
                            stf = (kWalkStops && (leaf_w >> 4) != kVoxelOffset) ? ST_PENDING : ST_LEAF;
                        } else {
                            mu0 = entry_magic<GE>(P0);
                            mu1 = entry_magic<GE>(P1);
                            mu2 = entry_magic<GE>(P2);
                            stf = ST_DESC;
                            if (CNT) satm = 0u;
                            restart_at(1u);
                        }
                    }
                }
                const uint32_t took = min(SHD ? 64u - (uint32_t)__popcll(act) : n_idle, pool_n);
                pool_i += took;
                pool_n -= took;
                act = __ballot(sabs(stf) >= ST_LEAF);
            }
            if (SHD && !more) {
                if (sabs(stf) == ST_PENDING) flush_record(true);
                act = __ballot(sabs(stf) >= ST_LEAF);
            }
            if (act == 0ull && pool_n == 0u && next == 0xFFFFFFFFu) break;
        }

        if (DBGH) {
            dbg_active += (uint32_t)__popcll(__ballot(sabs(stf) == ST_LEAF));
            const uint64_t now = __builtin_amdgcn_s_memtime();
            c_refill += (uint32_t)(now - c_mark);
            c_mark = now;
        }
        if (CNT) {
            const bool at_leaf = sabs(stf) == ST_LEAF && !(__uint_as_float(sh) < kMagic + (float)(D - SMAX));
            const uint64_t c_c0 = DBGH ? __builtin_amdgcn_s_memtime() : 0ull;
            if (__ballot(at_leaf) != 0ull) {
                const uint32_t L = (uint32_t)D - sh_of(sh);
                uint32_t todo = at_leaf ? (~satm & ((1u << L) - 2u)) : 0u;
                constexpr uint32_t kTopLv = (2u << K) - 2u;
                auto cell_k = [&](uint32_t x0, uint32_t x1, uint32_t x2) -> uint32_t {
                    return (__builtin_amdgcn_ubfe(x0, D - K, K) << (2 * K)) | (__builtin_amdgcn_ubfe(x1, D - K, K) << K) | __builtin_amdgcn_ubfe(x2, D - K, K);
// ... 28 lines not shown
                        if (l - 1u < (uint32_t)K) {
                            uint32_t x0 = mu0, x1 = mu1, x2 = mu2;
                            asm volatile("" : "+v"(x0), "+v"(x1), "+v"(x2));
                            const uint32_t cellK = cell_k(x0, x1, x2);
                            atomicOr(&top_sat[cellK >> 3], (1u << l) << ((cellK & 7u) * 4u));
                        }
                    }
                    cq_push(mine, p, 0u);
                }
            }
            if (DBGH) dbg_desc_start += (uint32_t)(__builtin_amdgcn_s_memtime() - c_c0);
        }
        if (sabs(stf) == ST_LEAF) {
            if (!kWalkStops && (leaf_w >> 4) != kVoxelOffset) {
                stf *= 0.5f;
            } else {
                const float Hm = __uint_as_float((sh << 23) + 0x3F000000u);
                const uint32_t keepm = 0xFFFFFFFFu << sh_of(sh), hbit = __float_as_uint(kMagic + Hm);
                auto t_axis = [&](uint32_t mu, float P, float Dr, float Y, float S) -> float {
                    const float c = __uint_as_float((mu & keepm) | hbit) - (kMagic + kScale);
                    return div_by_recip(__builtin_fmaf(S, Hm, c - P), Dr, Y);
                };
                const float t0 = t_axis(mu0, P0, Dr0, Y0, S0), t1 = t_axis(mu1, P1, Dr1, Y1, S1), t2 = t_axis(mu2, P2, Dr2, Y2, S2);
                const float tnew = __builtin_fminf(__builtin_fminf(t0, t1), t2);
                const float k0 = t0 == tnew ? kNudge : 0.0f, k1 = t1 == tnew ? kNudge : 0.0f, k2 = t2 == tnew ? kNudge : 0.0f;
                const float G0 = __builtin_fmaf(k0, S0, P0 + Dr0 * tnew);
                const float G1 = __builtin_fmaf(k1, S1, P1 + Dr1 * tnew);
                const float G2 = __builtin_fmaf(k2, S2, P2 + Dr2 * tnew);
                auto inside = [&](float G) -> float {
                    return __builtin_amdgcn_fmed3f(__builtin_fmaf(G, -4.0f, 4.0f * kScale), 0.0f, 1.0f) *
                           __builtin_amdgcn_fmed3f(__builtin_fmaf(G, 2.0f, 2.0f * kScale + 1.0f), 0.0f, 1.0f);
                };
                const float inbf = (inside(G0) * inside(G1)) * inside(G2);
                const float contf = inbf * __builtin_amdgcn_fmed3f(100.0f - stepsf, 0.0f, 1.0f);
                tcur = tnew;
                stepsf += inbf;
                nmf = __builtin_fmaf(k2, 4.0f, __builtin_fmaf(k1, 2.0f, k0));
                stf *= __builtin_fmaf(contf, 1.5f, 0.5f);
                if (contf > 0.5f) {
                    uint32_t n0, n1, n2;
                    if (GE) {
                        n0 = __float_as_uint(__builtin_floorf(G0) + (kScale + kMagic));
                        n1 = __float_as_uint(__builtin_floorf(G1) + (kScale + kMagic));
                        n2 = __float_as_uint(__builtin_floorf(G2) + (kScale + kMagic));
                    } else {
                        auto code_gt = [&](float G) -> uint32_t {
                            const float us = __builtin_amdgcn_fmed3f(__builtin_fmaf(__builtin_floorf(-G), -1.0f / kMagic, (kScale - 1.0f) / kMagic), 0.0f, 1.0f);
                            return __float_as_uint(__builtin_fmaf(us, kMagic, kMagic));
                        };
                        n0 = code_gt(G0); n1 = code_gt(G1); n2 = code_gt(G2);
                    }
                    const uint32_t lbit = __float_as_uint(__builtin_fmaf(Hm, 2.0f, kMagic)) & ((1u << D) - 1u);
                    const uint32_t diff = ((mu0 ^ n0) | (mu1 ^ n1) | (mu2 ^ n2)) | lbit;
                    mu0 = n0; mu1 = n1; mu2 = n2;
                    const uint32_t rb = (uint32_t)__builtin_clz(diff);
                    if (CNT) {
                        satm &= (1u << (rb - kRb)) - 1u;
                    }
                    restart_at_rb(rb);
                }
            }
        }
        if (DBGH) c_step += (uint32_t)(__builtin_amdgcn_s_memtime() - c_mark);
    }
    if (CNT) cq_flush();
    if (DBGH) {
#pragma unroll
        for (int o = 32; o > 0; o >>= 1) {
            dbg_desc_iters += (uint32_t)__shfl_xor((int)dbg_desc_iters, o);
            dbg_desc_lanes += (uint32_t)__shfl_xor((int)dbg_desc_lanes, o);
        }
    }
    if (DBGH) {
        uint32_t last = sabs(stf) == ST_PENDING ? (uint32_t)stepsf : 0u;
#pragma unroll
        for (int o = 32; o > 0; o >>= 1) last = max(last, (uint32_t)__shfl_xor((int)last, o));
        dbg_iters = last;
    }
    if (sabs(stf) == ST_PENDING) flush_record(false);
    {
        uint32_t *const bal = fresh_args().balance;
        if (bal != nullptr && tid == 0u && blockIdx.x < kBalanceSlots) bal[kBalanceHead + blockIdx.x] = (uint32_t)__builtin_amdgcn_s_memrealtime();
        if (bal != nullptr && tid == 0u && blockIdx.x == 0u) bal[kBalanceStamps] = gridDim.x;
    }
    if (DBG && lane == 0) {
        uint64_t t_end = __builtin_amdgcn_s_memrealtime();
        uint32_t *d = a.debug + 16u * wave_id;
        d[8] = c_refill;
        d[9] = c_desc;
        d[10] = c_step;
        d[11] = c_gen;
        d[12] = dbg_desc_iters;
        d[13] = dbg_desc_lanes;
        d[14] = dbg_desc_rounds;
        d[15] = dbg_desc_start;
        d[0] = t_begin;
        d[1] = t_dry ? t_dry : (uint32_t)t_end;
        d[2] = (uint32_t)t_end;
        d[3] = n_rounds;
        d[4] = dbg_active;
        d[5] = dbg_iters;
        d[6] = dbg_refills;
        d[7] = dbg_gens;
    }
}

constexpr uint32_t kScanChunk = 8192;

__device__ __forceinline__ void scan_classify(uint32_t node, bool &is_sub, bool &is_unsub) {
    const uint32_t counter = node & 15u;
    is_unsub = node != 0u && counter == 0u && (node >> 4) < kVoxelOffset;
    is_sub = node != 0u && !is_unsub && counter >= 4u && (node >> 4) > kVoxelOffset;
}

__global__ __launch_bounds__(256) void scan_kernel(uint32_t *nodes, uint32_t n_words, uint32_t node_length,
                                                   uint32_t *sub, uint32_t *unsub, uint32_t capacity, bool clear_counters) {
    __shared__ uint32_t tot[2][4];
    __shared__ uint32_t base[2];
    const uint32_t lane = threadIdx.x & 63u, wave = threadIdx.x >> 6;
    const uint32_t limit = min(n_words, node_length);
    auto load4 = [&](uint32_t id, uint32_t (&v)[4]) {
        if (id + 4u <= limit) {
            const uint4 q = *reinterpret_cast<const uint4 *>(nodes + id);
            v[0] = q.x; v[1] = q.y; v[2] = q.z; v[3] = q.w;
        } else {
#pragma unroll
            for (int k = 0; k < 4; k++) v[k] = (id + (uint32_t)k < limit) ? nodes[id + (uint32_t)k] : 0u;
        }
    };
    for (uint32_t chunk = blockIdx.x * kScanChunk; chunk < limit; chunk += gridDim.x * kScanChunk) {
        const uint32_t w0 = chunk + wave * (kScanChunk / 4u);
        uint32_t cs = 0, cu = 0;
        for (uint32_t it = 0; it < kScanChunk / 4u / 256u; it++) {
            uint32_t v[4];
            load4(w0 + it * 256u + lane * 4u, v);
#pragma unroll
            for (int k = 0; k < 4; k++) {
                bool a, b;
                scan_classify(v[k], a, b);
                cs += a ? 1u : 0u;
                cu += b ? 1u : 0u;
            }
        }
#pragma unroll
        for (int o = 32; o > 0; o >>= 1) {
            cs += (uint32_t)__shfl_xor((int)cs, o);
            cu += (uint32_t)__shfl_xor((int)cu, o);
        }
        if (lane == 0) { tot[0][wave] = cs; tot[1][wave] = cu; }
        __syncthreads();
        if (threadIdx.x < 2u) {
            uint32_t *list = threadIdx.x == 0u ? sub : unsub;
            const uint32_t n = tot[threadIdx.x][0] + tot[threadIdx.x][1] + tot[threadIdx.x][2] + tot[threadIdx.x][3];
            uint32_t b = capacity;
            if (n != 0u && __hip_atomic_load(&list[0], __ATOMIC_RELAXED, __HIP_MEMORY_SCOPE_AGENT) + 1u < capacity)
                b = atomicAdd(&list[0], n);
            base[threadIdx.x] = b;
        }
        __syncthreads();
        uint32_t bs = base[0], bu = base[1];
        for (uint32_t w = 0; w < wave; w++) { bs += tot[0][w]; bu += tot[1][w]; }
        const bool write_s = cs != 0u && (uint64_t)bs + 1u < capacity, write_u = cu != 0u && (uint64_t)bu + 1u < capacity;
        if (write_s || write_u || clear_counters) {
            for (uint32_t it = 0; it < kScanChunk / 4u / 256u; it++) {
                uint32_t v[4];
                const uint32_t id = w0 + it * 256u + lane * 4u;
                load4(id, v);
                if (clear_counters && ((v[0] | v[1] | v[2] | v[3]) & 15u)) {
                    if (id + 4u <= limit) {
                        *reinterpret_cast<uint4 *>(nodes + id) = make_uint4(v[0] & ~15u, v[1] & ~15u, v[2] & ~15u, v[3] & ~15u);
                    } else {
#pragma unroll
                        for (int k = 0; k < 4; k++)
                            if (id + (uint32_t)k < limit) nodes[id + (uint32_t)k] = v[k] & ~15u;
                    }
                }
#pragma unroll
                for (int k = 0; k < 4; k++) {
                    bool a, b;
                    scan_classify(v[k], a, b);
                    const uint64_t ms = __ballot(a), mu = __ballot(b);
                    if (write_s && ms) {
                        const uint32_t r = bs + __builtin_amdgcn_mbcnt_hi((uint32_t)(ms >> 32), __builtin_amdgcn_mbcnt_lo((uint32_t)ms, 0u));
                        if (a && (uint64_t)r + 1u < capacity) sub[1u + r] = id + (uint32_t)k;
                        bs += (uint32_t)__popcll(ms);
                    }
                    if (write_u && mu) {
// ... 193 lines not shown
        }
        c0 = powf(fmin_w(fmax_w(c0, 0.0f), 1.0f), gamma);
        c1 = powf(fmin_w(fmax_w(c1, 0.0f), 1.0f), gamma);
        c2 = powf(fmin_w(fmax_w(c2, 0.0f), 1.0f), gamma);
        const uint32_t r8 = (uint32_t)(c0 * 255.0f + 0.5f), g8 = (uint32_t)(c1 * 255.0f + 0.5f), b8 = (uint32_t)(c2 * 255.0f + 0.5f);
        rgba[it.out] = r8 | (g8 << 8) | (b8 << 16) | (128u << 24);
    }
}

hipError_t launch_secondary_gen(const TraceArgs &args, const float *aux_t, float *rays, uint8_t *skip, svo_hit *out, uint32_t k_first,
                                uint32_t n_secondary, uint32_t n_records, hipStream_t stream) {
    (void)hipGetLastError();
    uint32_t blocks = (args.work.n_items + 255u) / 256u;
    if (blocks > 4096u) blocks = 4096u;
    hipLaunchKernelGGL(secondary_gen_kernel, dim3(blocks), dim3(256), 0, stream, args, aux_t, rays, skip, out, k_first, n_secondary, n_records);
    return hipGetLastError();
}

hipError_t launch_shade(const TraceArgs &args, const svo_hit *shadow_hits, uint32_t *rgba, hipStream_t stream) {
    (void)hipGetLastError();
    uint32_t blocks = (args.work.n_items + 255u) / 256u;
    if (blocks > 4096u) blocks = 4096u;
    hipLaunchKernelGGL(shade_kernel, dim3(blocks), dim3(256), 0, stream, args, shadow_hits, rgba);
    return hipGetLastError();
}

__global__ __launch_bounds__(256) void diag_gather_kernel(const uint32_t *buf, uint32_t n_words, uint32_t stride_words,
                                                          uint32_t n_loads, uint32_t *sink) {
    const rsrc_t rs = make_rsrc(buf, n_words);
    uint32_t acc = 0;
    for (uint32_t i = blockIdx.x * 256u + threadIdx.x; i < n_loads; i += gridDim.x * 256u)
        acc += load_word(rs, i * stride_words);
    if (acc == 0x12345678u) *sink = acc;
}

hipError_t launch_diag_gather(const uint32_t *buf, uint32_t n_words, uint32_t stride_words, uint32_t n_loads, uint32_t *sink,
                              hipStream_t stream) {
    (void)hipGetLastError();
    hipLaunchKernelGGL(diag_gather_kernel, dim3(2048), dim3(256), 0, stream, buf, n_words, stride_words, n_loads, sink);
    return hipGetLastError();
}

hipError_t launch_build_top_table(const uint32_t *nodes, uint32_t n_words, uint32_t *top_table, hipStream_t stream) {
    (void)hipGetLastError();
    const int cells = 1 << (3 * kTopLevels);
    hipLaunchKernelGGL(build_top_table_kernel, dim3((cells + 255) / 256), dim3(256), 0, stream, nodes, n_words,
                       top_table, kTopLevels);
    return hipGetLastError();
}

constexpr int kStackBlock = 256;
constexpr int kStackLevels = 12;
constexpr int kStackLevelsDeep = 18;

int stack_max_depth(bool deep) { return kTopLevels + 1 + (deep ? kStackLevelsDeep : kStackLevels); }

template <bool GE, int NS>
static hipError_t launch_stack(const TraceArgs &args, const LaunchInfo &li, hipStream_t stream) {
    const uint32_t strip_items = args.order ? 64u : (li.strip_items ? li.strip_items : 64u);
    const bool shd = args.shadow_hits != nullptr;
    auto kern = shd ? (args.count_nodes ? trace_stack_kernel<kStackBlock, NS, kTopLevels, GE, false, true, true>
                                        : trace_stack_kernel<kStackBlock, NS, kTopLevels, GE, false, false, true>)
                    : (args.count_nodes
                           ? (args.debug ? trace_stack_kernel<kStackBlock, NS, kTopLevels, GE, true, true, false>
                                         : trace_stack_kernel<kStackBlock, NS, kTopLevels, GE, false, true, false>)
                           : (args.debug ? trace_stack_kernel<kStackBlock, NS, kTopLevels, GE, true, false, false>
                                         : trace_stack_kernel<kStackBlock, NS, kTopLevels, GE, false, false, false>));
    const size_t lds_bytes = sizeof(uint32_t) * (size_t)(args.count_nodes ? StackLds<kStackBlock, NS, kTopLevels, true>::total
                                                                               : StackLds<kStackBlock, NS, kTopLevels, false>::total);
    int &blocks_per_cu = li.occupancy[(args.debug ? 8 : 0) + (NS == kStackLevelsDeep ? 4 : 0) + (shd ? 2 : 0) + (args.count_nodes ? 1 : 0)];
    if (blocks_per_cu == 0) {
        int n = 0;
        hipError_t e = hipOccupancyMaxActiveBlocksPerMultiprocessor(&n, kern, kStackBlock, lds_bytes);
        if (e != hipSuccess) return e;
        blocks_per_cu = n > 0 ? n : 1;
        const int by_lds = (int)((160u * 1024u) / (((lds_bytes + 1279u) / 1280u) * 1280u));
        if (by_lds >= 1 && by_lds < blocks_per_cu) blocks_per_cu = by_lds;
    }
    uint32_t blocks = (uint32_t)li.num_cus * (uint32_t)blocks_per_cu;
    if (li.grid_blocks > 0) blocks = (uint32_t)li.grid_blocks;
    uint32_t n_strips = (args.work.n_items + strip_items - 1) / strip_items;
    uint32_t need = (n_strips + (kStackBlock / 64) - 1) / (kStackBlock / 64);
    if (blocks > need) blocks = need;
    hipLaunchKernelGGL(kern, dim3(blocks), dim3(kStackBlock), lds_bytes, stream, args, strip_items, li.counters, li.defer);
    return hipGetLastError();
}

hipError_t launch_trace(const TraceArgs &args, const LaunchInfo &li, hipStream_t stream) {
    (void)hipGetLastError();
    if (args.work.n_items == 0) return hipSuccess;
    const bool counter_hits = (args.u.flags & SVO_F_PAUSE_ADAPTIVE) && (args.u.flags & SVO_F_SHOW_HITS);
    if (li.variant == SVO_VARIANT_RESTART || counter_hits) {
        uint32_t blocks = (args.work.n_items + 255u) / 256u;
        uint32_t cap = (uint32_t)li.num_cus * 8u;
        if (li.grid_blocks > 0) cap = (uint32_t)li.grid_blocks;
        if (blocks > cap) blocks = cap;
        hipLaunchKernelGGL(trace_restart_kernel, dim3(blocks), dim3(256), 0, stream, args, (const uint32_t *)nullptr);
        return hipGetLastError();
    }
    const bool ge = (args.u.flags & SVO_F_MISC_BOOL) != 0;
    if (li.deep_stack)
        return ge ? launch_stack<true, kStackLevelsDeep>(args, li, stream) : launch_stack<false, kStackLevelsDeep>(args, li, stream);
    return ge ? launch_stack<true, kStackLevels>(args, li, stream) : launch_stack<false, kStackLevels>(args, li, stream);
}

hipError_t launch_post(const TraceArgs &args, const LaunchInfo &li, const PostPlan &plan, const SchedBuffers &buf, hipStream_t stream) {
    const uint32_t n_strips = (args.work.n_items + 63u) / 64u;
    uint8_t *const measure = plan.rebuild && !plan.reuse_costs ? buf.cost : nullptr;
    uint32_t blocks = measure ? (n_strips + 3u) / 4u : 256u;
    if (blocks > 2048u) blocks = 2048u;
    if (blocks < 16u) blocks = 16u;
    hipLaunchKernelGGL(post_kernel, dim3(blocks), dim3(256), 0, stream, args, li.counters, (const uint32_t *)li.defer,
                       li.next_defer_count, measure, n_strips, plan.balance_update);
    if (plan.build_lists) return launch_build_lists(args, plan.motion_floor, buf, stream);
    return hipGetLastError();
}

template <bool PACKED>
__global__ __launch_bounds__(256) void assemble_tiles_kernel(const uint32_t *gathered, uint4 *frame, uint32_t world, uint32_t n_pad,
                                                             uint32_t width, uint32_t height, uint32_t tile_w, uint32_t tile_h) {
    const uint32_t tiles_x = width / tile_w, n = width * height;
    for (uint32_t i = blockIdx.x * 256u + threadIdx.x; i < n; i += gridDim.x * 256u) {
        const uint32_t y = i / width, x = i - y * width;
        const uint32_t ty = y / tile_h, tx = x / tile_w;
        const uint32_t t = ty * tiles_x + tx, r = t % world, k = t / world;
        const uint64_t src = ((uint64_t)r * n_pad + k) * (tile_w * tile_h) + (y - ty * tile_h) * tile_w + (x - tx * tile_w);
        if (PACKED) {
            const uint32_t *p = gathered + 3u * src;
            const uint32_t info = p[2];
            frame[i] = make_uint4(p[0], p[1], info, (info >> 17) & 63u);
        } else {
            frame[i] = reinterpret_cast<const uint4 *>(gathered)[src];
        }
    }
}

__global__ __launch_bounds__(256) void pack_records_kernel(const uint4 *records, uint32_t *wire, uint32_t n) {
    for (uint32_t i = blockIdx.x * 256u + threadIdx.x; i < n; i += gridDim.x * 256u) {
        const uint4 r = records[i];
        wire[3u * i + 0u] = r.x;
        wire[3u * i + 1u] = r.y;
        wire[3u * i + 2u] = r.z;
    }
}

__global__ __launch_bounds__(256) void assemble_tiles_rgba_kernel(const uint32_t *gathered, uint32_t *frame, uint32_t world, uint32_t n_pad,
                                                                  uint32_t width, uint32_t height, uint32_t tile_w, uint32_t tile_h) {
    const uint32_t tiles_x = width / tile_w, n = width * height;
    for (uint32_t i = blockIdx.x * 256u + threadIdx.x; i < n; i += gridDim.x * 256u) {
        const uint32_t y = i / width, x = i - y * width;
        const uint32_t ty = y / tile_h, tx = x / tile_w;
        const uint32_t t = ty * tiles_x + tx, r = t % world, k = t / world;
        frame[i] = gathered[((uint64_t)r * n_pad + k) * (tile_w * tile_h) + (y - ty * tile_h) * tile_w + (x - tx * tile_w)];
    }
}

hipError_t launch_assemble_tiles_rgba(const uint32_t *gathered, uint32_t *frame, uint32_t world, uint32_t n_pad, uint32_t width,
                                      uint32_t height, uint32_t tile_w, uint32_t tile_h, hipStream_t stream) {
    (void)hipGetLastError();
    uint32_t blocks = (width * height + 255u) / 256u;
    if (blocks > 8192u) blocks = 8192u;
    hipLaunchKernelGGL(assemble_tiles_rgba_kernel, dim3(blocks), dim3(256), 0, stream, gathered, frame, world, n_pad, width, height, tile_w,
                       tile_h);
    return hipGetLastError();
}

// ... 54 lines not shown
```

octree-tracer_amd/gpu.py:

```python
import ctypes as C

import torch

from ._lib import SvoError, lib

OPT_VARIANT, OPT_TIMING, OPT_GRID_BLOCKS, OPT_REFILL_MIN, OPT_STRIP_ITEMS, OPT_DYNAMIC_STRIPS, OPT_PRIO_STEPS, OPT_DEBUG_BUFFER, OPT_SCHEDULE, OPT_TREE_DEPTH, OPT_BLOCK_SHAPE, OPT_SCAN_CLEARS_COUNTERS, OPT_FUSED_SHADOWS, OPT_PAIR_TABLE, OPT_CULL, OPT_CAMERA_SHORTCUT, OPT_SCHEDULE_MOTION = range(17)
VARIANT_RESTART, VARIANT_STACK = 0, 1


class Gpu:
    def __init__(self, device=0, stream=None):
        h = C.c_void_p()
        rc = lib().svo_ctx_create(device, C.byref(h))
        if rc != 0:
            raise SvoError(f"svo_ctx_create(device={device}) failed with status {rc} (no usable HIP device?)")
        self._h = h
        self.device = device
        self.torch_device = torch.device("cuda", device)
        self.tree_depth = 16
        self.set_stream(stream if stream is not None else torch.cuda.current_stream(device).cuda_stream)

    @classmethod
    def new(cls, device=0):
        return cls(device)

    def check(self, rc):
        if rc != 0:
            raise SvoError(f"status {rc}: {lib().svo_last_error(self._h).decode()}")

    def set_stream(self, hip_stream):
        self.check(lib().svo_ctx_set_stream(self._h, C.c_void_p(hip_stream), 0))

    def use_own_stream(self):
        self.check(lib().svo_ctx_set_stream(self._h, None, 1))

    def set_option(self, option, value):
        self.check(lib().svo_set_option(self._h, option, int(value)))
        if option == OPT_TREE_DEPTH:
            self.tree_depth = int(value)

    def declare_depth(self, depth, most=21):
        if 1 <= depth <= most and depth > self.tree_depth:
            self.set_option(OPT_TREE_DEPTH, depth)

    def sync(self):
        self.check(lib().svo_sync(self._h))

    def last_render_ms(self):
        ms = C.c_float()
        self.check(lib().svo_last_render_ms(self._h, C.byref(ms)))
        return ms.value

    def _timing(self, fn, n):
        ms = (C.c_float * n)()
        self.check(fn(self._h, ms))
        return list(ms)

    def build_timing(self):
        return self._timing(lib().svo_build_timing, 6)

    def edit_timing(self):
        return self._timing(lib().svo_edit_timing, 6)

    def compact_timing(self):
        return self._timing(lib().svo_compact_timing, 6)

    def list_timing(self):
        return self._timing(lib().svo_list_timing, 5)

    def sample_timing(self):
        return self._timing(lib().svo_sample_timing, 2)

    def voxelize_timing(self):
        return self._timing(lib().svo_voxelize_timing, 5)

    def world_build_timing(self):
        return self._timing(lib().svo_world_build_timing, 9)

    def strip_classes(self, n_strips):
        import numpy as np
        out = np.zeros(n_strips, dtype=np.uint8)
        self.check(lib().svo_diag_strip_classes(self._h, out.ctypes.data_as(C.c_void_p), n_strips))
        return out

    def timing_collect(self, cap=65536):
        import numpy as np
        buf = np.empty(cap, dtype=np.float32)
        n = C.c_size_t()
        self.check(lib().svo_timing_collect(self._h, buf.ctypes.data_as(C.POINTER(C.c_float)), cap, C.byref(n)))
        return buf[:n.value].copy()

    @staticmethod
    def comm_unique_id():
        buf = (C.c_uint8 * 128)()
        rc = lib().svo_comm_unique_id(buf)
        if rc != 0:
            raise SvoError(f"svo_comm_unique_id failed with status {rc} (librccl missing?)")
        return bytes(buf)

    def comm_init_rank(self, unique_id, world, rank):
        buf = (C.c_uint8 * 128).from_buffer_copy(unique_id)
        self.check(lib().svo_comm_init_rank(self._h, buf, world, rank))

    @staticmethod
    def comm_init_all(gpus):
        arr = (C.c_void_p * len(gpus))(*[g._h for g in gpus])
        rc = lib().svo_comm_init_all(len(gpus), arr)
        if rc != 0:
            raise SvoError(f"status {rc}: {lib().svo_last_error(gpus[0]._h).decode()}")

    def comm_destroy(self):
        self.check(lib().svo_comm_destroy(self._h))

    def gather_frame(self, send, recv_on_root=None, root=0):
        self.check(lib().svo_gather_frame(self._h, send.data_ptr(), send.numel() * send.element_size(),
                                          recv_on_root.data_ptr() if recv_on_root is not None else None, root))

    def gather_wait(self):
        self.check(lib().svo_gather_wait(self._h))

    def close(self):
        if getattr(self, "_h", None):
            lib().svo_ctx_destroy(self._h)
            self._h = None

    def __del__(self):
        if lib is not None:
            self.close()
```

Measured before the change: 9894.

## Replay a learned static per-wave strip deal instead of atomic work claiming

Adds a 'static deal' mode. When the camera and tree have not changed, each wave gets a precomputed table row of strips and walks it, with no atomic work-counter claims. The table is seeded from the stored schedule order lists. Per-wave start and end timestamps then drive a device-side learning step that moves strips from late waves to early ones across frames, with a compare kernel that keeps or reverts changes. This aims to remove atomic claim latency and tail imbalance in the persistent trace kernel, at the cost of extra small kernels, host-device state mirroring, and the risk of worse balance than dynamic claiming.

```diff
diff --git a/include/svo_hip.h b/include/svo_hip.h
--- a/include/svo_hip.h
+++ b/include/svo_hip.h
@@ -64,6 +64,7 @@
     SVO_OPT_CULL = 14,
     SVO_OPT_CAMERA_SHORTCUT = 15,
     SVO_OPT_SCHEDULE_MOTION = 16,
+    SVO_OPT_STATIC_DEAL = 17,
     SVO_OPT_PRIO_STEPS = 6
 } svo_option;
 
@@ -130,6 +131,9 @@
 
 int svo_diag_strip_classes(svo_ctx *ctx, uint8_t *host_out, size_t n_strips);
 
+int svo_diag_deal(svo_ctx *ctx, uint32_t status_out[16], uint32_t *table_out, size_t table_words, uint32_t *stamps_out,
+                  size_t stamps_words);
+
 int svo_scan_dispatch(svo_ctx *ctx, uint32_t node_length);
 int svo_scan_read(svo_ctx *ctx, uint32_t *sub, uint32_t *n_sub, uint32_t *unsub, uint32_t *n_unsub,
                   size_t capacity);
diff --git a/octree-tracer_amd/_lib.py b/octree-tracer_amd/_lib.py
--- a/octree-tracer_amd/_lib.py
+++ b/octree-tracer_amd/_lib.py
@@ -155,6 +155,7 @@
     "svo_timing_collect": (C.c_int, (vp, fp, sz, C.POINTER(sz))),
     "svo_diag_gather": (C.c_int, (vp, u32, u32)),
     "svo_diag_strip_classes": (C.c_int, (vp, vp, sz)),
+    "svo_diag_deal": (C.c_int, (vp, vp, vp, sz, vp, sz)),
     "svo_scan_dispatch": (C.c_int, (vp, u32)),
     "svo_scan_read": (C.c_int, (vp, vp, C.POINTER(u32), vp, C.POINTER(u32), sz)),
     "svo_proc_generate_chunk": (C.c_int, (vp, C.POINTER(ProcParams), C.POINTER(vp))),
diff --git a/octree-tracer_amd/csrc/svo_abi.cpp b/octree-tracer_amd/csrc/svo_abi.cpp
--- a/octree-tracer_amd/csrc/svo_abi.cpp
+++ b/octree-tracer_amd/csrc/svo_abi.cpp
@@ -176,13 +176,78 @@
     return SVO_OK;
 }
 
+int deal_before(svo_ctx *ctx, svo_ctx::Sched &sc, const svo::FrameFacts &ff, svo::TraceArgs &a, const svo::LaunchInfo &li, int sched_slot,
+                svo::DealPlan &plan) {
+    svo_ctx::Sched::DealBuffers &db = sc.deal;
+    svo::DealFacts f;
+    f.enabled = ctx->static_deal;
+    f.plain_static = sched_slot == 0 && a.work.mode != 2 && a.hits && !a.skip && !a.count_nodes && !a.shadow_hits && !a.debug && !li.deep_stack;
+    f.stored_lists = ff.schedule && !ff.filtered && a.order != nullptr && a.balance != nullptr;
+    f.at_rest = sc.built_nodes_version == ctx->store->version && memcmp(&sc.built_uniforms, &ctx->uniforms, sizeof(svo_uniforms)) == 0;
+    f.balance_frames = sc.state.balance_frames;
+    if (f.enabled && f.plain_static && f.stored_lists && f.at_rest) {
+        svo::LaunchInfo ask = li;
+        ask.blocks_out = &f.grid_blocks;
+        HIP_TRY(ctx, svo::launch_trace(a, ask, ctx->stream));
+        f.row_cap = svo::deal_row_cap(a.order_cap, f.grid_blocks);
+    }
+    if (db.seen_pending && hipEventQuery(db.seen_ev[0]) == hipSuccess) {
+        db.seen_pending = false;
+        f.seen_fresh = true;
+        f.seen_step = db.seen[svo::kDealStep];
+        f.seen_verdict = db.seen[svo::kDealVerdict];
+    }
+    (void)hipGetLastError();
+    const bool claimed_before = !db.last_replayed;
+    plan = svo::deal_before_trace(db.state, f);
+    db.last_replayed = plan.replay;
+    if (plan.seed) {
+        const size_t rows = (size_t)f.grid_blocks * 4;
+        if (int rc = svo_grow(ctx, rows * f.row_cap, &db.table)) return rc;
+        if (int rc = svo_grow(ctx, rows, &db.len)) return rc;
+        if (int rc = svo_grow(ctx, svo::deal_log_words(f.grid_blocks), &db.log)) return rc;
+        if (int rc = svo_grow(ctx, sc.order.size(), &db.lists)) return rc;
+        if (db.stamps.size() < 2 * rows) {
+            if (int rc = svo_grow(ctx, 2 * rows, &db.stamps)) return rc;
+            HIP_TRY(ctx, hipMemsetAsync(db.stamps, 0, db.stamps.size() * sizeof(uint32_t), ctx->stream));
+        }
+        if (!db.words) {
+            HIP_TRY(ctx, db.words.alloc(svo::kDealStateWords));
+            HIP_TRY(ctx, db.seen.alloc(svo::kDealStateWords));
+            HIP_TRY(ctx, db.seen_ev.create(hipEventDisableTiming));
+            HIP_TRY(ctx, hipMemsetAsync(db.words, 0, svo::kDealStateWords * sizeof(uint32_t), ctx->stream));
+            memset(db.seen, 0, svo::kDealStateWords * sizeof(uint32_t));
+        }
+        HIP_TRY(ctx, svo::launch_deal_seed(db.view(a.order_cap, ctx->deal_pairs_div), sc.order, claimed_before ? sc.balance.get() : nullptr, ctx->stream));
+    }
+    if (plan.replay) {
+        a.deal_table = db.table;
+        a.deal_row_cap = db.state.row_cap;
+        a.deal_stamps = db.stamps;
+    }
+    return SVO_OK;
+}
+
 int schedule_after(svo_ctx *ctx, svo_ctx::Sched &sc, svo::FrameFacts &f, const svo::TraceArgs &a, const svo::LaunchInfo &li,
-                   int sched_slot) {
+                   int sched_slot, const svo::DealPlan &deal) {
     f.same_input = (a.work.mode != 2 || sched_slot == 1) && sc.built_nodes_version == ctx->store->version &&
                    memcmp(&sc.built_uniforms, &ctx->uniforms, sizeof(svo_uniforms)) == 0;
     f.moving = sc.have_prev && memcmp(&sc.prev_uniforms, &ctx->uniforms, sizeof(svo_uniforms)) != 0;
-    const svo::PostPlan plan = svo::plan_after_trace(sc.state, f);
+    svo::PostPlan plan = svo::plan_after_trace(sc.state, f);
+    if (deal.replay) plan.balance_update = 0u;
     HIP_TRY(ctx, svo::launch_post(a, li, plan, sc.buf(), ctx->stream));
+    if (sched_slot == 0) {
+        svo_ctx::Sched::DealBuffers &db = sc.deal;
+        const svo::Deal view = db.view(a.order_cap, ctx->deal_pairs_div);
+        if (deal.step) HIP_TRY(ctx, svo::launch_deal_step(view, sc.balance, ctx->stream));
+        bool mirror = false;
+        if (svo::deal_after_post(db.state, deal, plan.build_lists, mirror)) HIP_TRY(ctx, svo::launch_deal_compare(view, sc.order, ctx->stream));
+        if (mirror) {
+            HIP_TRY(ctx, hipMemcpyAsync(db.seen, db.words, svo::kDealStateWords * sizeof(uint32_t), hipMemcpyDeviceToHost, ctx->stream));
+            HIP_TRY(ctx, hipEventRecord(db.seen_ev[0], ctx->stream));
+            db.seen_pending = true;
+        }
+    }
     sc.prev_uniforms = ctx->uniforms;
     sc.have_prev = true;
     if (plan.rebuild) {
@@ -263,6 +328,11 @@
         li.defer = lists + (ctx->frame_parity ? stride : 0);
         li.next_defer_count = lists + (ctx->frame_parity ? 0 : stride);
     }
+    svo::DealPlan deal;
+    if (stack) {
+        rc = deal_before(ctx, sc, f, a, li, opt.sched_slot, deal);
+        if (rc) return rc;
+    }
     const size_t slot = ctx->ev_slots ? (ctx->ev_count % ctx->ev_slots) : 0;
     const bool timed = ctx->ev_slots && opt.sched_slot == 0;
     if (timed) HIP_TRY(ctx, hipEventRecord(ctx->ev[slot][0], ctx->stream));
@@ -272,7 +342,7 @@
         ctx->ev_count++;
     }
     if (!stack) return SVO_OK;
-    rc = schedule_after(ctx, sc, f, a, li, opt.sched_slot);
+    rc = schedule_after(ctx, sc, f, a, li, opt.sched_slot, deal);
     if (rc) return rc;
     ctx->frame_parity ^= 1;
     return SVO_OK;
@@ -513,6 +583,10 @@
     if (!ctx) return SVO_ERR_HIP;
     ctx->device = hip_device;
     ctx->list_balance = getenv("SVO_NO_LIST_BALANCE") == nullptr;
+    if (const char *div = getenv("SVO_DEAL_PAIRS_DIV")) {
+        const long v = strtol(div, nullptr, 10);
+        if (v >= 2 && v <= 1024) ctx->deal_pairs_div = (uint32_t)v;
+    }
     hipError_t e = hipSetDevice(hip_device);
     hipDeviceProp_t prop;
     if (e == hipSuccess) e = hipGetDeviceProperties(&prop, hip_device);
@@ -626,6 +700,10 @@
         case SVO_OPT_PRIO_STEPS:
             if (value < 0 || value > 255) return svo_fail(ctx, SVO_ERR_ARG, "prio_steps must be 0..255");
             return SVO_OK;
+        case SVO_OPT_STATIC_DEAL:
+            if (value < 0 || value > 1) return svo_fail(ctx, SVO_ERR_ARG, "static deal: 0 (off) or 1 (on)");
+            ctx->static_deal = value != 0;
+            return SVO_OK;
         default:
             return svo_fail(ctx, SVO_ERR_ARG, "unknown option");
     }
@@ -897,6 +975,25 @@
     int rc = bind(ctx);
     if (rc) return rc;
     HIP_TRY(ctx, svo::launch_diag_gather(ctx->nodes, (uint32_t)ctx->capacity, stride_bytes / 4, n_loads, ctx->status, ctx->stream));
+    return SVO_OK;
+}
+
+int svo_diag_deal(svo_ctx *ctx, uint32_t status_out[16], uint32_t *table_out, size_t table_words, uint32_t *stamps_out, size_t stamps_words) {
+    if (!ctx || !status_out) return SVO_ERR_ARG;
+    int rc = bind(ctx);
+    if (rc) return rc;
+    const svo_ctx::Sched::DealBuffers &db = ctx->sched[0].deal;
+    uint32_t words[svo::kDealStateWords] = {};
+    HIP_TRY(ctx, hipStreamSynchronize(ctx->stream));
+    if (db.words) HIP_TRY(ctx, hipMemcpy(words, db.words, sizeof words, hipMemcpyDeviceToHost));
+    const uint32_t rows = db.state.seeded ? db.state.grid_blocks * 4u : 0u;
+    const uint32_t out[16] = {(uint32_t)db.state.replayed, (uint32_t)db.state.seeds, words[svo::kDealSeeds], words[svo::kDealMoves],
+                              words[svo::kDealStep], words[svo::kDealVerdict], db.state.seeded, db.state.claims, rows, db.state.row_cap,
+                              words[svo::kDealBestTime], words[svo::kDealBestSample], words[svo::kDealClaimTime], words[svo::kDealLastTime],
+                              words[svo::kDealLastMoves], db.state.learn_left};
+    memcpy(status_out, out, sizeof out);
+    if (table_out && rows) HIP_TRY(ctx, hipMemcpy(table_out, db.table, std::min(table_words, (size_t)rows * db.state.row_cap) * sizeof(uint32_t), hipMemcpyDeviceToHost));
+    if (stamps_out && rows) HIP_TRY(ctx, hipMemcpy(stamps_out, db.stamps, std::min(stamps_words, (size_t)rows * 2) * sizeof(uint32_t), hipMemcpyDeviceToHost));
     return SVO_OK;
 }
 
diff --git a/octree-tracer_amd/csrc/svo_ctx.h b/octree-tracer_amd/csrc/svo_ctx.h
--- a/octree-tracer_amd/csrc/svo_ctx.h
+++ b/octree-tracer_amd/csrc/svo_ctx.h
@@ -11,6 +11,7 @@
 #include <utility>
 #include <vector>
 
+#include "svo_deal.h"
 #include "svo_device.h"
 #include "svo_hip.h"
 #include "svo_host.h"
@@ -59,6 +60,10 @@
         for (int k = 0; k < N; k++) e[k] = o.e[k], o.e[k] = nullptr;
     }
     svo_events &operator=(const svo_events &) = delete;
+    svo_events &operator=(svo_events &&o) noexcept {
+        for (int k = 0; k < N; k++) std::swap(e[k], o.e[k]);
+        return *this;
+    }
     ~svo_events() { reset(); }
     void reset() {
         for (hipEvent_t &x : e) {
@@ -165,10 +170,24 @@
         uint64_t built_nodes_version = 0;
         svo_uniforms prev_uniforms{};
         bool have_prev = false;
+        struct DealBuffers {
+            svo::DealState state;
+            svo_dev<uint32_t> table, len, log, lists, stamps, words;
+            svo_pinned<uint32_t> seen;
+            svo_events<1> seen_ev;
+            bool seen_pending = false;
+            bool last_replayed = false;
+            svo::Deal view(uint32_t order_cap, uint32_t pairs_div) const {
+                return {table, len, log, lists, stamps, words, state.row_cap, state.grid_blocks, order_cap, pairs_div};
+            }
+        };
+        DealBuffers deal;
         hipError_t alloc(uint32_t n_strips);
         void release() { *this = Sched{}; }
     };
     Sched sched[2];
+    bool static_deal = true;
+    uint32_t deal_pairs_div = svo::kDealPairsDiv;
     bool list_balance = true;
     uint32_t motion_floor = 0x1204;
     bool schedule = true;
diff --git a/octree-tracer_amd/csrc/svo_deal.h b/octree-tracer_amd/csrc/svo_deal.h
--- /dev/null
+++ b/octree-tracer_amd/csrc/svo_deal.h
@@ -0,0 +1,317 @@
+#pragma once
+#include <cstddef>
+#include <cstdint>
+
+#include "svo_sched.h"
+
+#if defined(__HIPCC__) || defined(__CUDACC__)
+#define SVO_DEAL_HD __host__ __device__
+#else
+#define SVO_DEAL_HD
+#endif
+
+namespace svo {
+
+constexpr uint32_t kDealLearnFrames = 16;
+constexpr uint32_t kDealEnd = 0xFFFFFFFFu;
+constexpr uint32_t kDealMaxRow = 256;
+constexpr uint32_t kDealMaxListWaves = 1024;
+constexpr uint32_t kDealPairsDiv = 16;
+constexpr uint32_t kDealBalStart = 9, kDealBalStamps = 19, kDealBalBestTime = 20, kDealBalHead = 32, kDealBalSlots = 4096;
+
+enum : uint32_t {
+    kDealStep = 0,
+    kDealBestTime = 1,
+    kDealBestSample = 2,
+    kDealVerdict = 3,
+    kDealSeeds = 4,
+    kDealMoves = 5,
+    kDealLastTime = 6,
+    kDealLastMoves = 7,
+    kDealClaimTime = 8,
+    kDealBestStep = 9,
+    kDealTmpTime = 16,
+    kDealTmpSample = 17,
+    kDealTmpMoves = 18,
+    kDealStateWords = 32
+};
+
+struct Deal {
+    uint32_t *table;
+    uint32_t *len;
+    uint32_t *log;
+    uint32_t *lists;
+    uint32_t *stamps;
+    uint32_t *state;
+    uint32_t row_cap, grid_blocks, order_cap, pairs_div;
+};
+
+SVO_DEAL_HD inline uint32_t deal_list_waves(uint32_t grid_blocks, uint32_t l) { return ((grid_blocks + 7u - l) / 8u) * 4u; }
+SVO_DEAL_HD inline uint32_t deal_wave(uint32_t l, uint32_t rank) { return ((rank >> 2) * 8u + l) * 4u + (rank & 3u); }
+SVO_DEAL_HD inline uint32_t deal_log_slot(uint32_t grid_blocks, uint32_t s, uint32_t l, uint32_t p) {
+    uint32_t before = 0u;
+    for (uint32_t k = 0; k < l; k++) before += deal_list_waves(grid_blocks, k) / 2u;
+    return s * (grid_blocks * 2u) + before + p;
+}
+inline size_t deal_log_words(uint32_t grid_blocks) { return (size_t)kDealLearnFrames * grid_blocks * 2u * 2u; }
+
+inline uint32_t deal_row_cap(uint32_t order_cap, uint32_t grid_blocks) {
+    if (grid_blocks < 8u || deal_list_waves(grid_blocks, 0u) > kDealMaxListWaves) return 0u;
+    const uint32_t w_min = deal_list_waves(grid_blocks, 7u);
+    const uint32_t longest = (order_cap + w_min - 1u) / w_min;
+    uint32_t cap = 2u;
+    while (cap < 2u * longest + 1u) cap *= 2u;
+    return cap <= kDealMaxRow ? cap : 0u;
+}
+
+SVO_DEAL_HD inline bool deal_valid_time(uint32_t t) { return t != 0u && t < 100000000u; }
+
+template <typename Sync>
+SVO_DEAL_HD inline uint32_t deal_reduce_max(uint32_t *red, uint32_t mine, uint32_t tid, uint32_t nt, Sync sync) {
+    red[tid] = mine;
+    sync();
+    if (tid == 0u) {
+        uint32_t m = 0u;
+        for (uint32_t i = 0; i < nt; i++) m = red[i] > m ? red[i] : m;
+        red[0] = m;
+    }
+    sync();
+    const uint32_t m = red[0];
+    sync();
+    return m;
+}
+
+template <typename Sync>
+SVO_DEAL_HD inline uint32_t deal_sample_time(const uint32_t *bal, uint32_t *red, uint32_t tid, uint32_t nt, Sync sync) {
+    const uint32_t t0 = bal[kDealBalStart], n_slots = bal[kDealBalStamps] < kDealBalSlots ? bal[kDealBalStamps] : kDealBalSlots;
+    uint32_t mine = 0u;
+    for (uint32_t i = tid; i < n_slots; i += nt) {
+        const uint32_t t = bal[kDealBalHead + i] - t0;
+        if (deal_valid_time(t) && t > mine) mine = t;
+    }
+    return deal_reduce_max(red, mine, tid, nt, sync);
+}
+
+template <typename Sync>
+SVO_DEAL_HD inline void deal_seed(const Deal &d, const uint32_t *order, const uint32_t *bal, uint32_t *red, uint32_t tid, uint32_t nt, Sync sync) {
+    const uint32_t t_claims = bal ? deal_sample_time(bal, red, tid, nt, sync) : 0u;
+    for (uint32_t i = tid; i < 8u + 8u * d.order_cap; i += nt) d.lists[i] = order[i];
+    for (uint32_t l = 0; l < 8u; l++) {
+        const uint32_t w = deal_list_waves(d.grid_blocks, l);
+        const uint32_t len = order[l] < d.order_cap ? order[l] : d.order_cap;
+        for (uint32_t k = tid; k < len; k += nt) d.table[deal_wave(l, k % w) * d.row_cap + k / w] = order[8u + l * d.order_cap + k];
+        for (uint32_t r = tid; r < w; r += nt) {
+            const uint32_t n = len > r ? (len - r + w - 1u) / w : 0u;
+            d.table[deal_wave(l, r) * d.row_cap + n] = kDealEnd;
+            d.len[deal_wave(l, r)] = n;
+        }
+    }
+    if (tid == 0u) {
+        d.state[kDealStep] = 0u;
+        d.state[kDealBestTime] = d.state[kDealBestSample] = 0u;
+        d.state[kDealVerdict] = 0u;
+        d.state[kDealBestStep] = 0u;
+        d.state[kDealSeeds] += 1u;
+        if (bal) d.state[kDealClaimTime] = t_claims;
+    }
+    sync();
+}
+
+template <typename Sync>
+SVO_DEAL_HD inline void deal_reseed_if_changed(const Deal &d, const uint32_t *order, uint32_t *flag, uint32_t tid, uint32_t nt, Sync sync) {
+    if (tid == 0u) *flag = 0u;
+    sync();
+    bool differs = false;
+    for (uint32_t l = tid; l < 8u; l += nt) differs = differs || d.lists[l] != order[l];
+    for (uint32_t i = tid; i < 8u * d.order_cap; i += nt) {
+        const uint32_t l = i / d.order_cap, k = i - l * d.order_cap;
+        if (k < d.lists[l] && k < order[l]) differs = differs || d.lists[8u + i] != order[8u + i];
+    }
+    if (differs) *flag = 1u;
+    sync();
+    const bool reseed = *flag != 0u;
+    sync();
+    if (reseed) deal_seed(d, order, nullptr, nullptr, tid, nt, sync);
+}
+
+SVO_DEAL_HD inline void deal_move_last(const Deal &d, uint32_t from, uint32_t to) {
+    uint32_t *const rf = d.table + from * d.row_cap, *const rt = d.table + to * d.row_cap;
+    const uint32_t nf = d.len[from] - 1u, nt = d.len[to];
+    rt[nt] = rf[nf];
+    rt[nt + 1u] = kDealEnd;
+    rf[nf] = kDealEnd;
+    d.len[from] = nf;
+    d.len[to] = nt + 1u;
+}
+SVO_DEAL_HD inline bool deal_try_move(const Deal &d, uint32_t donor, uint32_t receiver, uint32_t t0, uint32_t slot) {
+    const int32_t end_d = (int32_t)(d.stamps[2u * donor + 1u] - t0), gen_d = (int32_t)(d.stamps[2u * donor] - t0);
+    const int32_t end_r = (int32_t)(d.stamps[2u * receiver + 1u] - t0);
+    const bool pays = end_d - end_r > end_d - gen_d && end_d - gen_d >= 0;
+    const bool ok = pays && d.len[donor] > 1u && d.len[receiver] + 2u <= d.row_cap;
+    if (ok) deal_move_last(d, donor, receiver);
+    d.log[2u * slot] = ok ? donor : kDealEnd;
+    d.log[2u * slot + 1u] = receiver;
+    return ok;
+}
+
+template <typename Sync>
+SVO_DEAL_HD inline void deal_step(const Deal &d, const uint32_t *bal, uint32_t *scratch, uint32_t l, uint32_t tid, uint32_t nt, Sync sync) {
+    const uint32_t n = d.state[kDealStep];
+    if (n >= kDealLearnFrames || d.state[kDealVerdict] != 0u) return;
+    const uint32_t best_before = d.state[kDealBestTime], t0 = bal[kDealBalStart];
+    const uint32_t n_rows = d.grid_blocks * 4u;
+    uint32_t *const t_of = scratch, *const by_rank = scratch + kDealMaxListWaves, *const red = scratch + 2u * kDealMaxListWaves;
+    uint32_t mine = 0u;
+    for (uint32_t w = tid; w < n_rows; w += nt) {
+        const uint32_t t = d.stamps[2u * w + 1u] - t0;
+        if (deal_valid_time(t) && t > mine) mine = t;
+    }
+    const uint32_t t_frame = deal_reduce_max(red, mine, tid, nt, sync);
+    const uint32_t t_sample = deal_sample_time(bal, red, tid, nt, sync);
+    const bool is_best = t_frame != 0u && (n == 0u || best_before == 0u || t_frame < best_before);
+    const bool last = n + 1u == kDealLearnFrames;
+    const uint32_t best_step = is_best ? n : d.state[kDealBestStep];
+    auto pairs_of = [&](uint32_t w) -> uint32_t {
+        uint32_t pairs = w / (d.pairs_div ? d.pairs_div : kDealPairsDiv);
+        pairs = pairs < 1u ? 1u : pairs;
+        return pairs > w / 2u ? w / 2u : pairs;
+    };
+    uint32_t moved = 0u;
+    if (last) {
+        for (uint32_t s = n; s-- > best_step;) {
+            for (uint32_t p = tid; p < pairs_of(deal_list_waves(d.grid_blocks, l)); p += nt) {
+                const uint32_t slot = deal_log_slot(d.grid_blocks, s, l, p);
+                if (d.log[2u * slot] != kDealEnd) deal_move_last(d, d.log[2u * slot + 1u], d.log[2u * slot]);
+            }
+            sync();
+        }
+    } else {
+        {
+            const uint32_t w = deal_list_waves(d.grid_blocks, l);
+            for (uint32_t i = tid; i < w; i += nt) t_of[i] = d.stamps[2u * deal_wave(l, i) + 1u] - t0;
+            sync();
+            for (uint32_t i = tid; i < w; i += nt) {
+                uint32_t r = 0u;
+                for (uint32_t j = 0; j < w; j++) r += (t_of[j] < t_of[i] || (t_of[j] == t_of[i] && j < i)) ? 1u : 0u;
+                by_rank[r] = i;
+            }
+            sync();
+            for (uint32_t p = tid; p < pairs_of(w); p += nt) {
+                if (t_frame == 0u) d.log[2u * deal_log_slot(d.grid_blocks, n, l, p)] = kDealEnd;
+                else moved += deal_try_move(d, deal_wave(l, by_rank[w - 1u - p]), deal_wave(l, by_rank[p]), t0, deal_log_slot(d.grid_blocks, n, l, p)) ? 1u : 0u;
+            }
+            sync();
+        }
+    }
+    red[tid] = moved;
+    sync();
+    if (tid == 0u) {
+        uint32_t m = 0u;
+        for (uint32_t i = 0; i < nt; i++) m += red[i];
+        d.state[kDealTmpMoves + l] = m;
+        if (l == 0u) {
+            d.state[kDealTmpTime] = t_frame;
+            d.state[kDealTmpSample] = t_sample;
+        }
+    }
+    sync();
+}
+
+SVO_DEAL_HD inline void deal_commit(const Deal &d, const uint32_t *bal) {
+    const uint32_t n = d.state[kDealStep];
+    if (n >= kDealLearnFrames || d.state[kDealVerdict] != 0u) return;
+    const uint32_t best_before = d.state[kDealBestTime], t_frame = d.state[kDealTmpTime];
+    const bool is_best = t_frame != 0u && (n == 0u || best_before == 0u || t_frame < best_before);
+    uint32_t m = 0u;
+    for (uint32_t l = 0; l < 8u; l++) m += d.state[kDealTmpMoves + l];
+    d.state[kDealMoves] += m;
+    d.state[kDealLastMoves] = m;
+    d.state[kDealLastTime] = t_frame;
+    if (is_best) {
+        d.state[kDealBestTime] = t_frame;
+        d.state[kDealBestSample] = d.state[kDealTmpSample];
+        d.state[kDealBestStep] = n;
+    }
+    d.state[kDealStep] = n + 1u;
+    if (n + 1u == kDealLearnFrames) {
+        const uint32_t learnt = bal[kDealBalBestTime], recent = d.state[kDealClaimTime], ours = d.state[kDealBestSample];
+        const uint32_t claims = learnt != 0u && (recent == 0u || learnt < recent) ? learnt : recent;
+        d.state[kDealVerdict] = (ours != 0u && (claims == 0u || ours < claims)) ? 1u : 2u;
+    }
+}
+
+
+struct DealFacts {
+    bool enabled = false;
+    bool plain_static = false;
+    bool stored_lists = false;
+    bool at_rest = false;
+    uint32_t balance_frames = 0;
+    uint32_t grid_blocks = 0, row_cap = 0;
+    uint32_t seen_step = 0, seen_verdict = 0;
+    bool seen_fresh = false;
+};
+
+struct DealState {
+    bool seeded = false;
+    bool claims = false;
+    uint32_t learn_left = 0;
+    uint32_t grid_blocks = 0, row_cap = 0;
+    bool want_mirror = false;
+    uint64_t replayed = 0, seeds = 0;
+};
+
+struct DealPlan {
+    bool seed = false;
+    bool replay = false;
+    bool step = false;
+    bool mirror = false;
+};
+
+inline DealPlan deal_before_trace(DealState &s, const DealFacts &f) {
+    DealPlan p;
+    const bool settled = f.at_rest && f.balance_frames >= kBalanceLearnFrames;
+    if (!(f.enabled && f.plain_static && f.stored_lists && settled && f.row_cap != 0u)) {
+        const uint64_t replayed = s.replayed, seeds = s.seeds;
+        s = DealState{};
+        s.replayed = replayed;
+        s.seeds = seeds;
+        return p;
+    }
+    if (f.seen_fresh && s.want_mirror) {
+        s.want_mirror = false;
+        if (f.seen_verdict == 2u) s.claims = true;
+        if (f.seen_step >= kDealLearnFrames) s.learn_left = 0;
+    }
+    if (!s.seeded || s.grid_blocks != f.grid_blocks || s.row_cap != f.row_cap) {
+        s.seeded = true;
+        s.claims = false;
+        s.learn_left = kDealLearnFrames;
+        s.grid_blocks = f.grid_blocks;
+        s.row_cap = f.row_cap;
+        s.want_mirror = false;
+        s.seeds++;
+        p.seed = true;
+    }
+    if (s.claims) return p;
+    p.replay = true;
+    s.replayed++;
+    if (s.learn_left != 0u) {
+        p.step = true;
+        s.learn_left--;
+        if (s.learn_left == 0u) p.mirror = s.want_mirror = true;
+    }
+    return p;
+}
+
+inline bool deal_after_post(DealState &s, const DealPlan &p, bool lists_rebuilt, bool &mirror) {
+    mirror = p.mirror;
+    if (!(s.seeded && lists_rebuilt)) return false;
+    if (!s.claims) {
+        s.learn_left = kDealLearnFrames;
+        mirror = s.want_mirror = true;
+    }
+    return !s.claims;
+}
+
+}
diff --git a/octree-tracer_amd/csrc/svo_deal.hip b/octree-tracer_amd/csrc/svo_deal.hip
--- /dev/null
+++ b/octree-tracer_amd/csrc/svo_deal.hip
@@ -0,0 +1,56 @@
+#include <hip/hip_runtime.h>
+
+#include "svo_deal.h"
+#include "svo_device.h"
+
+namespace svo {
+
+static_assert(kDealBalStart == kBalanceStart && kDealBalStamps == kBalanceStamps && kDealBalBestTime == kBalanceBestTime &&
+                  kDealBalHead == kBalanceHead && kDealBalSlots == kBalanceSlots,
+              "svo_deal.h reads the balance words by svo_device.h's numbers");
+
+constexpr uint32_t kDealThreads = 1024;
+
+struct BlockSync {
+    __device__ void operator()() const { __syncthreads(); }
+};
+
+__global__ __launch_bounds__(kDealThreads) void deal_seed_kernel(Deal d, const uint32_t *order, const uint32_t *bal) {
+    __shared__ uint32_t red[kDealThreads];
+    deal_seed(d, order, bal, red, threadIdx.x, kDealThreads, BlockSync{});
+}
+
+__global__ __launch_bounds__(kDealThreads) void deal_compare_kernel(Deal d, const uint32_t *order) {
+    __shared__ uint32_t flag;
+    deal_reseed_if_changed(d, order, &flag, threadIdx.x, kDealThreads, BlockSync{});
+}
+
+__global__ __launch_bounds__(kDealThreads) void deal_step_kernel(Deal d, const uint32_t *bal) {
+    __shared__ uint32_t scratch[2 * kDealMaxListWaves + kDealThreads];
+    deal_step(d, bal, scratch, blockIdx.x, threadIdx.x, kDealThreads, BlockSync{});
+}
+
+__global__ __launch_bounds__(64) void deal_commit_kernel(Deal d, const uint32_t *bal) {
+    if (threadIdx.x == 0u) deal_commit(d, bal);
+}
+
+hipError_t launch_deal_seed(const Deal &d, const uint32_t *order, const uint32_t *bal, hipStream_t stream) {
+    (void)hipGetLastError();
+    hipLaunchKernelGGL(deal_seed_kernel, dim3(1), dim3(kDealThreads), 0, stream, d, order, bal);
+    return hipGetLastError();
+}
+
+hipError_t launch_deal_compare(const Deal &d, const uint32_t *order, hipStream_t stream) {
+    (void)hipGetLastError();
+    hipLaunchKernelGGL(deal_compare_kernel, dim3(1), dim3(kDealThreads), 0, stream, d, order);
+    return hipGetLastError();
+}
+
+hipError_t launch_deal_step(const Deal &d, const uint32_t *bal, hipStream_t stream) {
+    (void)hipGetLastError();
+    hipLaunchKernelGGL(deal_step_kernel, dim3(8), dim3(kDealThreads), 0, stream, d, bal);
+    hipLaunchKernelGGL(deal_commit_kernel, dim3(1), dim3(64), 0, stream, d, bal);
+    return hipGetLastError();
+}
+
+}
diff --git a/octree-tracer_amd/csrc/svo_device.h b/octree-tracer_amd/csrc/svo_device.h
--- a/octree-tracer_amd/csrc/svo_device.h
+++ b/octree-tracer_amd/csrc/svo_device.h
@@ -54,6 +54,9 @@
     const uint8_t *skip;
     uint32_t *balance;
     svo_hit *shadow_hits;
+    const uint32_t *deal_table;
+    uint32_t deal_row_cap;
+    uint32_t *deal_stamps;
 };
 
 struct LaunchInfo {
@@ -66,6 +69,7 @@
     uint32_t *counters;
     uint32_t *defer;
     uint32_t *next_defer_count;
+    uint32_t *blocks_out;
 };
 
 hipError_t launch_build_top_table(const uint32_t *nodes, uint32_t n_words, uint32_t *top_table,
@@ -94,6 +98,11 @@
 hipError_t launch_post(const TraceArgs &args, const LaunchInfo &li, const PostPlan &plan, const SchedBuffers &buf, hipStream_t stream);
 hipError_t launch_build_lists(const TraceArgs &args, uint32_t motion_floor, const SchedBuffers &buf, hipStream_t stream);
 
+struct Deal;
+hipError_t launch_deal_seed(const Deal &d, const uint32_t *order, const uint32_t *bal, hipStream_t stream);
+hipError_t launch_deal_step(const Deal &d, const uint32_t *bal, hipStream_t stream);
+hipError_t launch_deal_compare(const Deal &d, const uint32_t *order, hipStream_t stream);
+
 hipError_t launch_schedule_skipping(const TraceArgs &args, const uint8_t *prev, uint8_t *cls, uint32_t *sched, uint32_t n_strips,
                                     uint32_t cap, hipStream_t stream);
 hipError_t launch_schedule_culling(const TraceArgs &args, const uint8_t *prev, uint8_t *cls, uint32_t *sched, uint32_t n_strips,
diff --git a/octree-tracer_amd/csrc/svo_kernels.hip b/octree-tracer_amd/csrc/svo_kernels.hip
--- a/octree-tracer_amd/csrc/svo_kernels.hip
+++ b/octree-tracer_amd/csrc/svo_kernels.hip
@@ -215,9 +215,9 @@
 #error "svo_kernels.hip is written for gfx950: the walk relies on its handling of LDS accesses beyond the allocation and on v_rcp_f32 + one Newton step being the IEEE reciprocal (tools/rcptest_gpu.hip)"
 #endif
 
-template <int BLOCK, int NS, int K, bool GE, bool DBG, bool CNT, bool SHD>
-__global__ __launch_bounds__(BLOCK, NS > 12 ? 4 : (CNT ? SVO_WAVES_PER_SIMD_CNT : ((SHD || (DBG && SVO_DBG_LIGHT == 0)) ? 6 : SVO_WAVES_PER_SIMD))) void trace_stack_kernel(TraceArgs a, uint32_t strip_items,
-                                                               uint32_t *work_counter, uint32_t *defer) {
+template <int BLOCK, int NS, int K, bool GE, bool DBG, bool CNT, bool SHD, bool REPLAY>
+__device__ __forceinline__ void trace_stack_body(const TraceArgs &a, uint32_t strip_items, uint32_t *work_counter, uint32_t *defer) {
+    static_assert(!REPLAY || (!DBG && !CNT && !SHD), "the replay kernel exists for the plain static frame only");
     constexpr bool DBGH = DBG && SVO_DBG_LIGHT == 0;
     constexpr int D = kPathBits;
     constexpr int SBASE = K + 2;
@@ -362,7 +362,7 @@
     static_assert(kShards * kSubs == 64, "the stealing probe reads one counter per lane");
     const uint32_t n_strips = (n_items + strip_items - 1) / strip_items;
     const uint32_t *order = a.order;
-    uint32_t home = (blockIdx.x % kShards) * kSubs + (blockIdx.x / kShards) % kSubs;
+    uint32_t home = REPLAY ? 0u : (blockIdx.x % kShards) * kSubs + (blockIdx.x / kShards) % kSubs;
     uint32_t pend = 0;
     uint32_t next, strip_end;
     auto entry_of = [=](uint32_t sh, uint32_t k) -> uint32_t {
@@ -370,7 +370,15 @@
         const uint32_t cand = (((k >> 4) * kShards + sh) << 4) | (k & 15u);
         return cand < n_strips ? cand : 0xFFFFFFFFu;
     };
-    {
+    auto row_entry = [=](uint32_t j) -> uint32_t {
+        const TraceArgs &fa = fresh_args();
+        return fa.deal_table[wave_id * fa.deal_row_cap + j];
+    };
+    if (REPLAY) {
+        const uint32_t s0 = __builtin_amdgcn_readfirstlane(row_entry(0u));
+        next = s0 != 0xFFFFFFFFu ? s0 * strip_items : 0xFFFFFFFFu;
+        strip_end = s0 != 0xFFFFFFFFu ? min(next + strip_items, n_items) : 0xFFFFFFFFu;
+    } else {
         const uint32_t my_rank = (blockIdx.x / kShards) * (uint32_t)(BLOCK / 64) + __builtin_amdgcn_readfirstlane(tid >> 6);
         const uint32_t s0 = __builtin_amdgcn_readfirstlane(entry_of(blockIdx.x % kShards, my_rank));
         if (s0 != 0xFFFFFFFFu) {
@@ -692,8 +700,8 @@
                     dbg_desc_rounds += (uint32_t)(__builtin_amdgcn_s_memtime() - c_w0);
                 }
                 uint32_t lst = home / kSubs;
-                uint32_t s = entry_of(lst, __builtin_amdgcn_readfirstlane(pend) * kSubs + home % kSubs + ((gridDim.x + kShards - 1u - lst) / kShards) * (uint32_t)(BLOCK / 64));
-                while (s == 0xFFFFFFFFu) {
+                uint32_t s = REPLAY ? pend : entry_of(lst, __builtin_amdgcn_readfirstlane(pend) * kSubs + home % kSubs + ((gridDim.x + kShards - 1u - lst) / kShards) * (uint32_t)(BLOCK / 64));
+                while (!REPLAY && s == 0xFFFFFFFFu) {
                     if (DBG && !DBGH && lane == 0u) dbg_desc_iters += 1u;
                     const uint32_t l = lane / kSubs;
                     const uint32_t cv = __hip_atomic_load(work_counter + lane * kShardStride, __ATOMIC_RELAXED, __HIP_MEMORY_SCOPE_AGENT);
@@ -714,7 +722,7 @@
                     if (lane == 0) k = atomicAdd(work_counter + home * kShardStride, 1u);
                     s = entry_of(lst, __builtin_amdgcn_readfirstlane(k) * kSubs + home % kSubs + ((gridDim.x + kShards - 1u - lst) / kShards) * (uint32_t)(BLOCK / 64));
                 }
-                home = (home & ~(kSubs - 1u)) | ((home + 1u) & (kSubs - 1u));
+                if (!REPLAY) home = (home & ~(kSubs - 1u)) | ((home + 1u) & (kSubs - 1u));
                 s = __builtin_amdgcn_readfirstlane(s);
                 next = s != 0xFFFFFFFFu ? s * strip_items : 0xFFFFFFFFu;
                 strip_end = s != 0xFFFFFFFFu ? min(next + strip_items, n_items) : 0xFFFFFFFFu;
@@ -732,6 +740,7 @@
                     }
                     const uint64_t c_g0 = DBGH ? __builtin_amdgcn_s_memtime() : 0ull;
                     const TraceArgs &a = fresh_args();
+                    if (REPLAY && lane == 0u) a.deal_stamps[2u * wave_id] = (uint32_t)__builtin_amdgcn_s_memrealtime();
                     const uint32_t q = next + lane;
                     bool alive = false;
                     float gp0 = 0, gp1 = 0, gp2 = 0, gd0 = 1, gd1 = 1, gd2 = 1, gdist = 0;
@@ -785,7 +794,12 @@
                     pool_i = 0u;
                     next += min(64u, strip_end - next);
                     if (next >= strip_end) {
-                        if (lane == 0) pend = atomicAdd(work_counter + home * kShardStride, 1u);
+                        if (REPLAY) {
+                            home += 1u;
+                            pend = row_entry(home);
+                        } else if (lane == 0) {
+                            pend = atomicAdd(work_counter + home * kShardStride, 1u);
+                        }
 #ifdef SVO_PROBE_CLAIM_LATENCY
                         if (DBG) {
                             const uint64_t c_a0 = __builtin_amdgcn_s_memtime();
@@ -980,6 +994,7 @@
         uint32_t *const bal = fresh_args().balance;
         if (bal != nullptr && tid == 0u && blockIdx.x < kBalanceSlots) bal[kBalanceHead + blockIdx.x] = (uint32_t)__builtin_amdgcn_s_memrealtime();
         if (bal != nullptr && tid == 0u && blockIdx.x == 0u) bal[kBalanceStamps] = gridDim.x;
+        if (REPLAY && lane == 0u) fresh_args().deal_stamps[2u * wave_id + 1u] = (uint32_t)__builtin_amdgcn_s_memrealtime();
     }
     if (DBG && lane == 0) {
         uint64_t t_end = __builtin_amdgcn_s_memrealtime();
@@ -1001,6 +1016,17 @@
         d[6] = dbg_refills;
         d[7] = dbg_gens;
     }
+}
+
+template <int BLOCK, int NS, int K, bool GE, bool DBG, bool CNT, bool SHD>
+__global__ __launch_bounds__(BLOCK, NS > 12 ? 4 : (CNT ? SVO_WAVES_PER_SIMD_CNT : ((SHD || (DBG && SVO_DBG_LIGHT == 0)) ? 6 : SVO_WAVES_PER_SIMD))) void trace_stack_kernel(TraceArgs a, uint32_t strip_items,
+                                                               uint32_t *work_counter, uint32_t *defer) {
+    trace_stack_body<BLOCK, NS, K, GE, DBG, CNT, SHD, false>(a, strip_items, work_counter, defer);
+}
+
+template <int BLOCK, int NS, int K, bool GE>
+__global__ __launch_bounds__(BLOCK, SVO_WAVES_PER_SIMD) void trace_stack_replay_kernel(TraceArgs a, uint32_t strip_items, uint32_t *defer) {
+    trace_stack_body<BLOCK, NS, K, GE, false, false, false, true>(a, strip_items, nullptr, defer);
 }
 
 constexpr uint32_t kScanChunk = 8192;
@@ -1360,6 +1386,19 @@
     uint32_t n_strips = (args.work.n_items + strip_items - 1) / strip_items;
     uint32_t need = (n_strips + (kStackBlock / 64) - 1) / (kStackBlock / 64);
     if (blocks > need) blocks = need;
+    if (li.blocks_out) {
+        *li.blocks_out = blocks;
+        return hipSuccess;
+    }
+    if (args.deal_table != nullptr) {
+        if constexpr (NS == kStackLevels) {
+            if (shd || args.count_nodes || args.debug) return hipErrorInvalidValue;
+            hipLaunchKernelGGL((trace_stack_replay_kernel<kStackBlock, NS, kTopLevels, GE>), dim3(blocks), dim3(kStackBlock), lds_bytes, stream, args,
+                               strip_items, li.defer);
+            return hipGetLastError();
+        }
+        return hipErrorInvalidValue;
+    }
     hipLaunchKernelGGL(kern, dim3(blocks), dim3(kStackBlock), lds_bytes, stream, args, strip_items, li.counters, li.defer);
     return hipGetLastError();
 }
diff --git a/octree-tracer_amd/gpu.py b/octree-tracer_amd/gpu.py
--- a/octree-tracer_amd/gpu.py
+++ b/octree-tracer_amd/gpu.py
@@ -4,7 +4,7 @@
 
 from ._lib import SvoError, lib
 
-OPT_VARIANT, OPT_TIMING, OPT_GRID_BLOCKS, OPT_REFILL_MIN, OPT_STRIP_ITEMS, OPT_DYNAMIC_STRIPS, OPT_PRIO_STEPS, OPT_DEBUG_BUFFER, OPT_SCHEDULE, OPT_TREE_DEPTH, OPT_BLOCK_SHAPE, OPT_SCAN_CLEARS_COUNTERS, OPT_FUSED_SHADOWS, OPT_PAIR_TABLE, OPT_CULL, OPT_CAMERA_SHORTCUT, OPT_SCHEDULE_MOTION = range(17)
+OPT_VARIANT, OPT_TIMING, OPT_GRID_BLOCKS, OPT_REFILL_MIN, OPT_STRIP_ITEMS, OPT_DYNAMIC_STRIPS, OPT_PRIO_STEPS, OPT_DEBUG_BUFFER, OPT_SCHEDULE, OPT_TREE_DEPTH, OPT_BLOCK_SHAPE, OPT_SCAN_CLEARS_COUNTERS, OPT_FUSED_SHADOWS, OPT_PAIR_TABLE, OPT_CULL, OPT_CAMERA_SHORTCUT, OPT_SCHEDULE_MOTION, OPT_STATIC_DEAL = range(18)
 VARIANT_RESTART, VARIANT_STACK = 0, 1
 
 
@@ -83,6 +83,26 @@
         self.check(lib().svo_diag_strip_classes(self._h, out.ctypes.data_as(C.c_void_p), n_strips))
         return out
 
+    DEAL_STATUS = ("replayed", "seeds", "device_seeds", "moves", "step", "verdict", "seeded", "claims", "rows", "row_cap",
+                   "best_ticks", "best_sample_ticks", "claim_ticks", "last_ticks", "last_moves", "learn_left")
+
+    def deal_status(self, table=False, stamps=False):
+        import numpy as np
+        st = np.zeros(16, dtype=np.uint32)
+        self.check(lib().svo_diag_deal(self._h, st.ctypes.data_as(C.c_void_p), None, 0, None, 0))
+        out = dict(zip(self.DEAL_STATUS, (int(v) for v in st)))
+        rows, cap = out["rows"], out["row_cap"]
+        tab = np.zeros((rows, cap), dtype=np.uint32) if table else None
+        stp = np.zeros((rows, 2), dtype=np.uint32) if stamps else None
+        if rows and (table or stamps):
+            self.check(lib().svo_diag_deal(self._h, st.ctypes.data_as(C.c_void_p), tab.ctypes.data_as(C.c_void_p) if table else None,
+                                           tab.size if table else 0, stp.ctypes.data_as(C.c_void_p) if stamps else None, stp.size if stamps else 0))
+        if table:
+            out["table"] = tab
+        if stamps:
+            out["stamps"] = stp
+        return out
+
     def timing_collect(self, cap=65536):
         import numpy as np
         buf = np.empty(cap, dtype=np.float32)
```

Result: faster. 10880 (median of 6 runs) (+9.9%).
